# gvanhorn38/multibox

Measured on AMD Instinct MI355X. Metric: images/sec (299x299, 5-AR priors) train, higher is better.
Workload: dtype bf16; 1 GPU; full train step: Inception-ResNet-v2 + multibox heads fwd, on-device matching+loss, bwd, RMSProp+EMA; 299x299, k=5 (P=646), BATCH_SIZE=64/GPU, MAX_NUM_BBOXES=13; global_batch=64, parallelism=dp1, hip_graph=True

## Files before the change

### include/mbx.h

```cpp
#ifndef MBX_H
#define MBX_H

#include <stddef.h>
#include <stdint.h>

#ifdef __cplusplus
extern "C" {
#endif

typedef void* mbx_stream_t;

typedef enum {
  MBX_OK = 0,
  MBX_ERR_INVALID_ARG = -1,
  MBX_ERR_UNSUPPORTED = -2,
  MBX_ERR_LAUNCH = -3,
  MBX_ERR_WORKSPACE = -4
} mbx_status;

int mbx_version(void);
const char* mbx_status_string(int status);

int mbx_priors_count(int k, const int* grids, int n_grids);

// ... 9 lines not shown
size_t mbx_match_workspace_bytes(int B, int P, int G);
int mbx_match(const float* decoded , const float* conf ,
              const float* gt , const int32_t* n_gt , float alpha,
              int B, int P, int G, int32_t* match , int32_t* status ,
              void* workspace, size_t workspace_bytes, mbx_stream_t stream);

int mbx_match_extend(const float* priors , const float* gt ,
                     const int32_t* n_gt , const int32_t* status ,
                     float iou_threshold, int B, int P, int G,
                     int32_t* match ,
                     int32_t* n_extra , mbx_stream_t stream);

size_t mbx_loss_workspace_bytes(int B);
int mbx_loss_fwd_bwd(const float* decoded , const float* conf_in ,
                     int conf_is_logit, const float* gt ,
                     const int32_t* match , float alpha, float grad_scale, int B, int P,
                     int G, float* loss2 ,
                     float* d_raw_locs , float* d_logits ,
                     void* workspace, size_t workspace_bytes, mbx_stream_t stream);

size_t mbx_loss_mined_workspace_bytes(int B, int P);
int mbx_loss_fwd_bwd_mined(const float* decoded , const float* conf_in ,
                           int conf_is_logit, const float* gt ,
                           const int32_t* match , float alpha, float grad_scale, int B, int P,
                           int G, float* loss2 ,
                           float* d_raw_locs , float* d_logits ,
                           int neg_per_pos, int min_neg, int32_t* n_neg ,
                           void* workspace, size_t workspace_bytes, mbx_stream_t stream);

size_t mbx_loss_focal_workspace_bytes(int B, int P);
int mbx_loss_fwd_bwd_focal(const float* decoded , const float* conf_in ,
                           int conf_is_logit, const float* gt ,
                           const int32_t* match , float alpha, float grad_scale, int B, int P,
                           int G, float* loss2 ,
                           float* d_raw_locs , float* d_logits ,
                           float gamma, float w_pos, float w_neg,
                           int neg_per_pos , int min_neg, int32_t* n_neg ,
                           void* workspace, size_t workspace_bytes, mbx_stream_t stream);

enum { MBX_LOC_L2 = 0, MBX_LOC_SMOOTH_L1 = 1, MBX_LOC_GIOU = 2, MBX_LOC_DIOU = 3, MBX_LOC_CIOU = 4 };
size_t mbx_loss_loc_workspace_bytes(int B, int P);
int mbx_loss_fwd_bwd_loc(const float* decoded , const float* conf_in ,
                         int conf_is_logit, const float* gt ,
                         const int32_t* match , float alpha, float grad_scale, int B, int P,
                         int G, float* loss2 ,
                         float* d_raw_locs , float* d_logits ,
                         int loc_type , float loc_beta ,
                         float gamma, float w_pos, float w_neg,
                         int neg_per_pos , int min_neg, int32_t* n_neg ,
                         void* workspace, size_t workspace_bytes, mbx_stream_t stream);

typedef struct {
  int32_t offset_y, offset_x;
  int32_t patch_h, patch_w;
  int32_t image_h, image_w;
  int32_t is_flipped;
  int32_t max_to_keep;
  float restrictions[4];
} mbx_patch_meta;

int mbx_decode_filter_topk(const float* raw_locs , const float* conf ,
                           const float* priors , const mbx_patch_meta* meta ,
                           int B, int P, int k_max, double* out_boxes ,
                           float* out_scores , int32_t* out_index ,
                           int32_t* out_count , mbx_stream_t stream);

int mbx_nms(double* boxes , float* scores , int32_t* index ,
            int32_t* count , int B, int k_max, double iou_threshold, mbx_stream_t stream);

#define MBX_MERGE_MAX_CANDIDATES 16384
int mbx_merge_detections(const double* boxes , const float* scores ,
                         const int32_t* count , const int32_t* image_rows , int I, int k_max,
                         int max_det, double iou_threshold, double* out_boxes ,
                         float* out_scores , int32_t* out_src ,
                         int32_t* out_count , int32_t* out_status , mbx_stream_t stream);

int mbx_merge_detections_voted(const double* boxes , const float* scores ,
                               const int32_t* count , const int32_t* image_rows , int I,
                               int k_max, int max_det, double iou_threshold, double vote_iou_threshold,
                               double* out_boxes , float* out_scores ,
                               int32_t* out_src , int32_t* out_count ,
                               int32_t* out_status , int32_t* out_votes , mbx_stream_t stream);

#define MBX_SOFT_LINEAR 1
#define MBX_SOFT_GAUSSIAN 2
int mbx_merge_detections_soft(const double* boxes , const float* scores ,
                              const int32_t* count , const int32_t* image_rows , int I, int k_max,
                              int max_det, int method, double iou_threshold , double sigma ,
                              double min_score, double vote_iou_threshold ,
                              double* out_boxes , float* out_scores ,
                              int32_t* out_src , int32_t* out_count , int32_t* out_status ,
                              int32_t* out_votes , mbx_stream_t stream);

#define MBX_COCO_MAX_DET 100
#define MBX_COCO_MAX_GT 128
int mbx_coco_match(const double* dt , const int32_t* dt_rows ,
                   const double* gt , const int32_t* gt_rows , int I,
                   const double* iou_thrs , int T, const double* area_rng ,
                   int A, int16_t* match , uint8_t* ignore ,
                   int32_t* n_gt_counted , int32_t* status , mbx_stream_t stream);

#define MBX_COCO_ACC_MAX_R 128
#define MBX_COCO_ACC_MAX_M 4
#define MBX_COCO_ACC_MAX_ND 4194304
#define MBX_COCO_ACC_CHUNK 256
#define MBX_COCO_ACC_SORT_TILE 1024
size_t mbx_coco_accumulate_workspace(long long ND, int T, int A, int M);
int mbx_coco_accumulate(const double* dt , const int32_t* dt_rows , int I,
                        const int16_t* match , const uint8_t* ignore ,
                        const int32_t* n_gt_counted , int T, int A, const double* rec_thrs , int R,
                        const int32_t* max_dets , int M, double* precision ,
                        double* recall , void* workspace, size_t workspace_bytes, mbx_stream_t stream);

typedef enum {
  MBX_EPI_STORE = 0,
  MBX_EPI_AFFINE = 1,
  MBX_EPI_RESIDUAL = 2,
  MBX_EPI_STORE_F32 = 3
} mbx_epilogue;

typedef struct {
  int32_t n, rows_mod;
  int32_t c_begin[4];
  const void* y[4]; int32_t ld_y[4];
  const float* relu_thr[4];
  float* stats[4]; int32_t stats_ld[4];
} mbx_bn_bwd_stats;

#define MBX_GRID_BARRIER_BYTES 6400
typedef struct {
  void* barrier;
  void* a; int32_t ld_a;
  const float* beta;
  float* mean; float* rstd;
  float* moving_mean; float* moving_var;
  float* relu_thr;
  int32_t relu; float eps, decay;
  float* step_poison;
} mbx_bn_apply_desc;

#define MBX_BN_BWD_SLOTS 8
typedef struct {
  void* barrier;
  int32_t n;
  int32_t c_begin[4];
  const void* y[4]; int32_t ld_y[4];
  void* dy[4]; int32_t ld_dy[4];
  const float* mean[4]; const float* rstd[4]; const float* beta[4];
  float* dbeta[4];
  float* acc[4]; int32_t acc_ld[4];
  int32_t relu[4];
  float* step_poison;
} mbx_bn_bwd_fused;

typedef struct {
  const void* x; int64_t x_img_stride; int32_t ldx;
  int32_t N, H_in, W_in, C_in;
  const void* w; int32_t C_out, R, S;
  int32_t stride, transposed, pad_t, pad_l, H_out, W_out;
  void* y; int64_t y_img_stride; int32_t ldy;
  int32_t epilogue, relu, accumulate;
  const float* scale; const float* shift;
  const void* skip; int64_t skip_img_stride; int32_t ld_skip; float rscale;
  float* stats_partial;
  int32_t tile_config;
  const void* acc_src; int64_t acc_img_stride; int32_t ld_acc;
  int32_t* work_counter;
  int32_t max_workgroups;
  void* splitk_ws; int64_t splitk_ws_bytes;
  int32_t stats_rows_mod, stats_ld;
  const mbx_bn_bwd_stats* bn_bwd_stats;
  void* relu_bits; int32_t ld_bits;
  const mbx_bn_apply_desc* bn_apply;
  const mbx_bn_bwd_fused* bn_bwd;
} mbx_conv_desc;
#define MBX_CONV_TILE_CONFIGS 14
#define MBX_TILE_I5_BASE 32
#define MBX_TILE_I7 65
#define MBX_TILE_DIRECT3 96
#define MBX_TILE_DIRECTW 97
#define MBX_TILE_RESIDENT 98
#define MBX_TILE_PWRES 99
#define MBX_TILE_SPLITK_BASE 128
#define MBX_TILE_SPLITK_MAX 32

int mbx_conv_stats_rows(const mbx_conv_desc* desc );
int mbx_conv(const mbx_conv_desc* desc , mbx_stream_t stream);
int mbx_conv_supported(const mbx_conv_desc* desc );
int mbx_conv_pair(const mbx_conv_desc* a , const mbx_conv_desc* b , mbx_stream_t stream);
size_t mbx_conv_splitk_workspace_bytes(const mbx_conv_desc* desc );

int mbx_conv_wgrad(const mbx_conv_desc* desc , const void* dy,
                   int64_t dy_img_stride, int32_t ld_dy, float* dw, float* db, mbx_stream_t stream);

typedef struct {
  mbx_conv_desc desc;
  const void* dy; int64_t dy_img_stride; int32_t ld_dy;
  float scale;
  float* dw; float* db;
} mbx_wgrad_job;
typedef struct {
  int32_t n_layers, n_items;
  int64_t layers_off, items_off;
  int64_t queues_off, heads_off;
  double flops;
  int64_t tally_off;
} mbx_wgrad_plan_info;
#define MBX_WGRAD_DETERMINISTIC 1
#define MBX_WGRAD_SCATTER 2
size_t mbx_wgrad_plan_bytes(const mbx_wgrad_job* jobs , int n_jobs, int flags);
int mbx_wgrad_plan(const mbx_wgrad_job* jobs , int n_jobs, int flags, void* host_image, size_t bytes,
                   mbx_wgrad_plan_info* info );
int mbx_conv_wgrad_grouped(void* device_image , const mbx_wgrad_plan_info* info ,
                           mbx_stream_t stream);
int mbx_conv_wgrad_grouped_capped(void* device_image, const mbx_wgrad_plan_info* info , int max_workgroups,
                                  mbx_stream_t stream);

int mbx_conv_wgrad_scaled(const mbx_conv_desc* desc, const void* dy, int64_t dy_img_stride,
                          int32_t ld_dy, float scale, float* dw, float* db, mbx_stream_t stream);

int mbx_bn_finalize(const float* stats_partial , int rows, int C, int64_t count,
                    float eps, float decay, float* mean , float* rstd ,
                    float* moving_mean , float* moving_var ,
                    mbx_stream_t stream);
int mbx_bn_apply(const void* y, int64_t M, int C, const float* mean, const float* rstd,
                 const float* beta, int relu, void* a, int ld_a, mbx_stream_t stream);
int mbx_bn_apply_fused(const float* stats_partial, int rows, int64_t count, float eps, float decay,
                       const void* y, int64_t M, int C, const float* beta, int relu, void* a, int ld_a,
                       float* mean, float* rstd, float* moving_mean, float* moving_var,
                       mbx_stream_t stream);
int mbx_bn_apply_fused_mapped(const void* stats_fixed, int rows, int64_t count, float eps, float decay,
                              const void* y, int64_t M, int C, const float* beta, int relu, void* a, int ld_a,
                              const struct mbx_chan_map_s* a_map , float* mean, float* rstd, float* moving_mean,
                              float* moving_var, float* relu_thr, mbx_stream_t stream);
int mbx_bn_moving_update(float* moving_mean, float* moving_var, const float* batch_mean, const float* batch_var,
                         int64_t n, float decay, const float* skip_ctl, uint64_t* skipped_steps,
                         float* ema_mean, float* ema_var, float ema_decay, mbx_stream_t stream);
typedef struct mbx_chan_map_s { int32_t n; int32_t c_begin[4]; int32_t offset[4]; } mbx_chan_map;
int mbx_bn_finalize_parts(const float* const* parts , const int32_t* rows ,
                          const int32_t* Cs , int n_parts, int64_t count, float eps, float decay, float* mean,
                          float* rstd, float* moving_mean, float* moving_var, mbx_stream_t stream);
int mbx_bn_apply_mapped(const void* y, int64_t M, int C, const float* mean, const float* rstd, const float* beta,
                        int relu, void* a, int ld_a, const mbx_chan_map* a_map , mbx_stream_t stream);
int mbx_bn_apply_maxpool(const void* y, int N, int H, int W, int C, const float* mean, const float* rstd, const float* beta,
                         int relu, void* p, int64_t p_img_stride, int ld_p, int Ho, int Wo, uint8_t* argmax,
                         mbx_stream_t stream);
int mbx_bn_fold(const float* moving_mean, const float* moving_var, const float* beta, float eps,
                int C, float* scale, float* shift, mbx_stream_t stream);
int mbx_bn_bwd_rows(int64_t M, int C);
int mbx_bn_bwd_reduce(const void* da, int ld_da, const void* a, int ld_a, int relu, const void* y,
                      int64_t M, int C, const float* mean, const float* rstd, const float* beta,
                      float* partial , mbx_stream_t stream);
int mbx_bn_bwd_finalize(const float* partial, int rows, int C, int64_t M, float* dbeta ,
                        float* m12 , mbx_stream_t stream);
int mbx_bn_bwd_apply(const void* da, int ld_da, const void* a, int ld_a, int relu, const void* y,
                     int64_t M, int C, const float* mean, const float* rstd, const float* beta,
                     const float* m12, void* dy , mbx_stream_t stream);

int mbx_bn_bwd_reduce_mapped(const void* da, int ld_da, const void* a, int ld_a, int relu, const void* y, int64_t M, int C,
                             const float* mean, const float* rstd, const float* beta, float* partial,
                             const mbx_chan_map* da_map , mbx_stream_t stream);
int mbx_bn_bwd_apply_mapped(const void* da, int ld_da, const void* a, int ld_a, int relu, const void* y, int64_t M, int C,
                            const float* mean, const float* rstd, const float* beta, const float* m12, void* dy,
                            const mbx_chan_map* da_map , mbx_stream_t stream);

int mbx_bn_bwd_apply_rows(const float* stats, int rows, const void* da, int ld_da, const void* y, int64_t M, int C,
                          const float* mean, const float* rstd, const float* relu_thr, float* dbeta, void* dy,
                          const mbx_chan_map* da_map , mbx_stream_t stream);

size_t mbx_bn_bwd_onepass_workspace_bytes(int C);
int mbx_bn_bwd_onepass_supported(int64_t M, int C, int max_workgroups);
int mbx_bn_bwd_onepass(const void* da, int ld_da, int relu, const void* y, int64_t M, int C,
                       const float* mean, const float* rstd, const float* beta, float* dbeta ,
                       void* dy , void* ws, int max_workgroups, float* step_poison ,
                       mbx_stream_t stream);

int mbx_bn_bwd_rows_pooled(int N, int H, int W, int C);
int mbx_bn_bwd_reduce_pooled(const void* gy, int64_t gy_img_stride, int ld_gy, const uint8_t* argmax, int N, int H, int W,
                             int Ho, int Wo, int relu, const void* y, int C, const float* mean, const float* rstd,
                             const float* beta, float* partial , mbx_stream_t stream);
int mbx_bn_bwd_apply_pooled(const void* gy, int64_t gy_img_stride, int ld_gy, const uint8_t* argmax, int N, int H, int W,
                            int Ho, int Wo, int relu, const void* y, int C, const float* mean, const float* rstd,
                            const float* beta, const float* m12, void* dy, mbx_stream_t stream);
int mbx_bn_bwd_onepass_mapped(const void* da, int ld_da, int relu, const void* y, int64_t M, int C, const float* mean,
                              const float* rstd, const float* beta, float* dbeta, void* dy, void* ws, int max_workgroups,
                              float* step_poison, const mbx_chan_map* da_map , mbx_stream_t stream);

int mbx_maxpool_fwd(const void* x, int64_t x_img_stride, int ldx, int N, int H, int W, int C,
                    int k, int stride, void* y, int64_t y_img_stride, int ldy, int Ho, int Wo,
                    uint8_t* argmax , mbx_stream_t stream);
int mbx_maxpool_bwd(const void* dy, int64_t dy_img_stride, int ld_dy, const uint8_t* argmax,
                    int N, int H, int W, int C, int k, int stride, int Ho, int Wo, void* dx,
                    int64_t dx_img_stride, int ld_dx, int accumulate, mbx_stream_t stream);
int mbx_avgpool_fwd(const void* x, int64_t x_img_stride, int ldx, int N, int H, int W, int C,
                    int k, int pad, void* y, int64_t y_img_stride, int ldy, int Ho, int Wo,
                    mbx_stream_t stream);
int mbx_avgpool_bwd(const void* dy, int64_t dy_img_stride, int ld_dy, int N, int H, int W, int C,
                    int k, int pad, int Ho, int Wo, void* dx, int64_t dx_img_stride, int ld_dx,
                    int accumulate, mbx_stream_t stream);

int mbx_relu_mask(void* g, int ld_g, const void* a, int ld_a, int64_t M, int C, mbx_stream_t stream);
int mbx_pack_input(const float* img, int64_t pixels, void* out, mbx_stream_t stream);
int mbx_head_gather(const float* h, int ld_h, int N, int cells, int k, int P, int off,
                    float* locs, float* logits, mbx_stream_t stream);
int mbx_head_scatter(const float* d_locs, const float* d_logits, int N, int cells, int k, int P,
                     int off, void* g, int ld_g, mbx_stream_t stream);

typedef struct {
  const float* h; int32_t ld_h;
  void* g; int32_t ld_g;
  int32_t cells, k, off;
} mbx_head;
int mbx_head_gather_all(const mbx_head* heads , int n_heads, int N, int P, float* locs, float* logits,
                        mbx_stream_t stream);
int mbx_head_scatter_all(const float* d_locs, const float* d_logits, const mbx_head* heads , int n_heads, int N,
                         int P, mbx_stream_t stream);

int mbx_step_begin(float* grads, int64_t n_grads, float* bn_ws, int64_t n_ws, int64_t ctl_index, uint64_t* timeouts_total,
                   float* zero_scalar, mbx_stream_t stream);

typedef struct {
  int64_t src_off;
  int64_t dst_off;
  int32_t K, R, S, C, Kpad;
  int32_t first_block;
} mbx_filter_entry;
int mbx_filter_prepare(const void* w_bf16, void* w_dgrad, const mbx_filter_entry* table ,
// ... 56 lines not shown
```

### multibox_amd/csrc/conv.hip

```cpp
#include <stdlib.h>

#include "conv_common.h"

namespace {

template <int BM, int BN, int WNW, int WMW, int EV, int MODE = 0, int NSTG = 3>
__device__ __forceinline__ void conv_igemm3_body(const ConvK& p, const int bid_, const int nblk_) {
  constexpr bool SH = MODE == 2, PW = MODE == 1;
  static_assert(WNW * WMW == 4 || WNW * WMW == 8, "four or eight waves");
  constexpr int NT = 64 * WNW * WMW, RPP = NT / 8;
  constexpr int TN = BN / WNW, TM = BM / WMW, NI = TN / 16, MI = TM / 16;
  constexpr int PI = BM / RPP, WI = BN / RPP, NL = PI + WI;
  constexpr int STAGE = (BM + BN) * 8;
  extern __shared__ __attribute__((aligned(16))) u32x4 smem[];

  const int tid = threadIdx.x, lane = tid & 63;
  const int wave = wave_id();
  const int wn = wave % WNW, wm = wave / WNW;
  int lid = xcd_remap(bid_, nblk_);
  int split = 0;
  if constexpr (EV == 5) { const int nt = p.tiles_m * p.tiles_n; split = lid / nt; lid -= split * nt; }
  const int tile_n = lid % p.tiles_n, tile_m = lid / p.tiles_n;
  const int m0 = tile_m * BM, n0 = tile_n * BN;

// ... 394 lines not shown
  return MBX_OK;
}

}

extern "C" int mbx_conv_stats_rows(const mbx_conv_desc* d) {
  if (!d) return MBX_ERR_INVALID_ARG;
  if (d->stats_rows_mod > 0) return d->stats_rows_mod;
  const long M = (long)d->N * d->H_out * d->W_out;
  if (d->tile_config > kSplitFlag) return (int)((M + kSplitRows - 1) / kSplitRows);
  if (d->tile_config == kDirectCfg) return mbx_direct3_grid(d->N, d->H_out, d->W_out);
  if (d->tile_config == kDirectWCfg) { const int g = mbx_directw_grid(d->N, d->H_out, d->W_out); return g > 0 ? g : MBX_ERR_UNSUPPORTED; }
  if (d->tile_config == kResidentCfg) return mbx_resident_rows(d->N);
  if (d->tile_config == kI7Cfg) return (int)((M + 127) / 128);
  if (d->tile_config > kI5Flag) {
    const int i = d->tile_config - kI5Flag - 1;
    if (i >= mbx_i5_num_tiles) return MBX_ERR_INVALID_ARG;
    return (int)((M + mbx_i5_tiles[i][0] - 1) / mbx_i5_tiles[i][0]);
  }
  const TileCfg& c = kCfgs[choose_cfg(M, d->C_out, d->tile_config)];
  return (int)((M + c.BM - 1) / c.BM);
}

static int conv_impl(const mbx_conv_desc* d, mbx_stream_t stream, int dry);
extern "C" int mbx_conv(const mbx_conv_desc* d, mbx_stream_t stream) { return conv_impl(d, stream, 0); }
extern "C" int mbx_conv_supported(const mbx_conv_desc* d) { return conv_impl(d, nullptr, 1); }
extern "C" int mbx_conv_pair(const mbx_conv_desc* a, const mbx_conv_desc* b, mbx_stream_t stream) {
  PairCapture ca, cb;
  g_capture.valid = 0;
  int st = conv_impl(a, stream, 2);
  if (st != MBX_OK) return st;
  if (!g_capture.valid) return MBX_ERR_UNSUPPORTED;
  ca = g_capture;
  g_capture.valid = 0;
  st = conv_impl(b, stream, 2);
  if (st != MBX_OK) return st;
  if (!g_capture.valid) return MBX_ERR_UNSUPPORTED;
  cb = g_capture;
  if (ca.bm != cb.bm || ca.bn != cb.bn || ca.wnw != cb.wnw || ca.wmw != cb.wmw || ca.nstg != cb.nstg || ca.ev != cb.ev ||
      ca.mode != 0 || cb.mode != 0 || (ca.ev != 0 && ca.ev != 1 && ca.ev != 6) || ca.wnw != 2 || ca.wmw != 2 || ca.bn != 64)
    return MBX_ERR_UNSUPPORTED;
  ca.k.dry = cb.k.dry = 0;
  hipStream_t s = mbx_s(stream);
#define MBX_PAIR(BM_, NSTG_)                                                                                      \
  if (ca.bm == BM_ && ca.nstg == NSTG_)                                                                           \
    return ca.ev == 6 ? launch_pair_inst<BM_, 64, 2, 2, 6, NSTG_>(ca.k, cb.k, s)                                    \
           : ca.ev ? launch_pair_inst<BM_, 64, 2, 2, 1, NSTG_>(ca.k, cb.k, s) : launch_pair_inst<BM_, 64, 2, 2, 0, NSTG_>(ca.k, cb.k, s);
  MBX_PAIR(128, 2) MBX_PAIR(128, 3) MBX_PAIR(64, 2) MBX_PAIR(64, 3)
#undef MBX_PAIR
  return MBX_ERR_UNSUPPORTED;
}

extern "C" size_t mbx_conv_splitk_workspace_bytes(const mbx_conv_desc* d) {
  if (!d || d->tile_config <= kSplitFlag || d->tile_config > kSplitFlag + kSplitMax) return 0;
  int ksplit, kps;
  splitk_geom((d->R * d->S * d->C_in + 63) >> 6, d->tile_config - kSplitFlag, ksplit, kps);
  return (size_t)4 * d->N * d->H_out * d->W_out * (((d->C_out + 7) / 8) * 8) * ksplit;
}

static int conv_impl(const mbx_conv_desc* d, mbx_stream_t stream, int dry) {
  int st = check_desc(d);
  if (st != MBX_OK) return st;
  if (!d->w || !d->y) return MBX_ERR_INVALID_ARG;
  if ((reinterpret_cast<uintptr_t>(d->w) & 15)) return MBX_ERR_INVALID_ARG;
  const bool f32 = d->epilogue == MBX_EPI_STORE_F32;
  if (!f32 && (d->C_out % 8 || d->ldy % 8 || (reinterpret_cast<uintptr_t>(d->y) & 15))) return MBX_ERR_INVALID_ARG;
  if (d->epilogue == MBX_EPI_RESIDUAL && (!d->skip || d->ld_skip % 8 || (reinterpret_cast<uintptr_t>(d->skip) & 15)))
    return MBX_ERR_INVALID_ARG;
  if ((long long)d->N * d->y_img_stride >= (1LL << 31)) return MBX_ERR_UNSUPPORTED;
  if (d->stats_partial && (d->epilogue != MBX_EPI_STORE || d->accumulate || d->skip)) return MBX_ERR_INVALID_ARG;
  if (d->epilogue == MBX_EPI_STORE && d->skip && (d->ld_skip % 8 || (reinterpret_cast<uintptr_t>(d->skip) & 15))) return MBX_ERR_INVALID_ARG;
  MBX_ENTER();
  ConvK k;
  k.x = reinterpret_cast<const unsigned short*>(d->x);
  k.x_img_stride = (int)d->x_img_stride; k.ldx = d->ldx; k.H_in = d->H_in; k.W_in = d->W_in; k.C_in = d->C_in;
  k.w = reinterpret_cast<const unsigned short*>(d->w);
  k.C_out = d->C_out; k.R = d->R; k.S = d->S; k.Ktot = d->R * d->S * d->C_in;
  k.x_bytes = (unsigned)(2 * ((long long)(d->N - 1) * d->x_img_stride + ((long long)d->H_in * d->W_in - 1) * d->ldx + d->C_in));
  k.w_bytes = (unsigned)(2LL * d->C_out * k.Ktot);
  if (d->transposed) { k.mul = 1; k.shift = d->stride == 2 ? 1 : 0; } else { k.mul = d->stride; k.shift = 0; }
  k.pad_t = d->pad_t; k.pad_l = d->pad_l; k.W_out = d->W_out; k.HW_out = d->H_out * d->W_out;
  k.M = d->N * k.HW_out;
  k.y = d->y; k.y_img_stride = (int)d->y_img_stride; k.ldy = d->ldy;
  k.epi = d->epilogue; k.relu = d->relu; k.accumulate = d->accumulate;
  k.scale = d->scale; k.shiftv = d->shift;
  k.skip = reinterpret_cast<const unsigned short*>(d->skip);
  k.skip_img_stride = (int)d->skip_img_stride; k.ld_skip = d->ld_skip; k.rscale = d->rscale;
  k.bits = nullptr; k.bits_ld = 0; k.bits_bytes = 0;
  if (d->relu_bits) {
    const bool wr = d->epilogue == MBX_EPI_RESIDUAL && d->relu, rd = d->epilogue == MBX_EPI_STORE && !d->skip;
    if ((!wr && !rd) || d->ld_bits % 4 || d->ld_bits < 4 * ((d->C_out + 31) / 32) || (reinterpret_cast<uintptr_t>(d->relu_bits) & 3)) return MBX_ERR_INVALID_ARG;
    if (d->stats_partial || d->bn_bwd_stats) return MBX_ERR_UNSUPPORTED;
    const long long bb = (long long)d->N * d->H_out * d->W_out * d->ld_bits;
    if (bb >= (1LL << 31)) return MBX_ERR_UNSUPPORTED;
    k.bits = reinterpret_cast<unsigned char*>(d->relu_bits); k.bits_ld = d->ld_bits; k.bits_bytes = (unsigned)bb;
  }
  k.stats = d->stats_partial;
  if (d->stats_rows_mod < 0 || d->stats_rows_mod > 1024 || d->stats_ld < 0 || (d->stats_ld && d->stats_ld < d->C_out)) return MBX_ERR_INVALID_ARG;
  k.stats_mod = d->stats_rows_mod; k.stats_ld = d->stats_ld ? d->stats_ld : d->C_out;
  k.stats_cap = 0.f;
  k.fa = FusedApply{};
  k.fa.bar = nullptr;
  k.fb = FusedBwd{};
  k.fb.bar = nullptr;
  if (d->bn_bwd) {
    const mbx_bn_bwd_fused* b = d->bn_bwd;
    if (!b->barrier || (reinterpret_cast<uintptr_t>(b->barrier) & 127) || b->n < 1 || b->n > 4 || b->c_begin[0] != 0) return MBX_ERR_INVALID_ARG;
    if (d->epilogue != MBX_EPI_STORE || d->accumulate || d->skip || d->relu_bits || d->stats_partial || d->bn_bwd_stats || d->bn_apply ||
        d->stride != 1 || d->C_out > 2048 || d->y_img_stride != (int64_t)d->H_out * d->W_out * d->ldy)
      return MBX_ERR_UNSUPPORTED;
    const int tc = d->tile_config;
    if (!((tc > kI5Flag && tc <= kI5Flag + 7) || tc == kDirectWCfg || tc == kResidentCfg)) return MBX_ERR_UNSUPPORTED;
    const long long Mll = (long long)d->N * d->H_out * d->W_out;
    for (int i = 0; i < 4; ++i) k.fb.cb[i] = 1 << 30;
    for (int i = 0; i < b->n; ++i) {
      if (!b->y[i] || !b->dy[i] || !b->mean[i] || !b->rstd[i] || (b->relu[i] && !b->beta[i]) || !b->acc[i] ||
          (reinterpret_cast<uintptr_t>(b->y[i]) & 15) || (reinterpret_cast<uintptr_t>(b->dy[i]) & 15) || b->ld_y[i] % 8 || b->ld_dy[i] % 8 ||
          b->c_begin[i] % 8 || b->c_begin[i] >= d->C_out || (i && b->c_begin[i] <= b->c_begin[i - 1]) || b->acc_ld[i] <= 0)
        return MBX_ERR_INVALID_ARG;
      if (Mll * b->ld_y[i] >= (1LL << 31) || Mll * b->ld_dy[i] >= (1LL << 31)) return MBX_ERR_UNSUPPORTED;
      k.fb.cb[i] = b->c_begin[i];
      k.fb.y[i] = reinterpret_cast<const unsigned short*>(b->y[i]); k.fb.ldy[i] = b->ld_y[i];
      k.fb.dy[i] = reinterpret_cast<unsigned short*>(b->dy[i]); k.fb.lddy[i] = b->ld_dy[i];
      k.fb.mean[i] = b->mean[i]; k.fb.rstd[i] = b->rstd[i]; k.fb.beta[i] = b->beta[i]; k.fb.dbeta[i] = b->dbeta[i];
      k.fb.acc[i] = b->acc[i]; k.fb.acc_ld[i] = b->acc_ld[i]; k.fb.relu[i] = b->relu[i];
    }
    const int fault = mbx_barrier_fault() == '3';
    k.fb.n = b->n;
    k.fb.bar = reinterpret_cast<unsigned*>(b->barrier);
    static const int probe = mbx_env_int("MBX_FUSED_PROBE", 0) & ~1;
    k.fb.spin_limit = fault ? (1u << 10) : (1u << 22); k.fb.fault = fault | probe; k.fb.step_poison = b->step_poison;
    k.fb.inv_M = (float)(1.0 / (double)Mll);
  }
  if (d->bn_apply) {
    const mbx_bn_apply_desc* b = d->bn_apply;
    if (!b->barrier || !b->a || !b->beta || !b->mean || !b->rstd || (reinterpret_cast<uintptr_t>(b->barrier) & 127) ||
        (reinterpret_cast<uintptr_t>(b->a) & 15) || b->ld_a % 8 || b->ld_a < d->C_out)
      return MBX_ERR_INVALID_ARG;
    if (!d->stats_partial || d->stats_rows_mod < 1 || d->stats_rows_mod > 16 || d->epilogue != MBX_EPI_STORE || d->accumulate || d->skip ||
        d->transposed || d->rscale != 0.f || d->C_out > 2048 || d->y_img_stride != (int64_t)d->H_out * d->W_out * d->ldy ||
        (long long)d->N * d->H_out * d->W_out * b->ld_a >= (1LL << 31))
      return MBX_ERR_UNSUPPORTED;
    const int tc = d->tile_config;
    if (!((tc > kI5Flag && tc <= kI5Flag + 7) || tc == kDirectWCfg || tc == kResidentCfg)) return MBX_ERR_UNSUPPORTED;
    const int fault = mbx_barrier_fault() == '2';
    k.fa.bar = reinterpret_cast<unsigned*>(b->barrier);
    static const int probe = mbx_env_int("MBX_FUSED_PROBE", 0) & ~1;
    k.fa.spin_limit = fault ? (1u << 10) : (1u << 22); k.fa.fault = fault | probe; k.fa.step_poison = b->step_poison;
    k.fa.a = reinterpret_cast<unsigned short*>(b->a); k.fa.ld_a = b->ld_a; k.fa.beta = b->beta;
    k.fa.mean = b->mean; k.fa.rstd = b->rstd; k.fa.mmean = b->moving_mean; k.fa.mvar = b->moving_var; k.fa.thr = b->relu_thr;
    k.fa.relu = b->relu; k.fa.eps = b->eps; k.fa.decay = b->decay;
    k.fa.inv_count = 1.0 / (double)((long long)d->N * d->H_out * d->W_out);
  }
  k.bw_n = 0; k.bw_mod = 1;
  for (int i = 0; i < 4; ++i) { k.bw_cb[i] = 1 << 30; k.bw_ldy[i] = 0; k.bw_sld[i] = 0; k.bw_y[i] = nullptr; k.bw_thr[i] = nullptr; k.bw_stats[i] = nullptr; }
  if (d->bn_bwd_stats) {
    const mbx_bn_bwd_stats* b = d->bn_bwd_stats;
    if (d->epilogue != MBX_EPI_STORE || d->accumulate || d->skip || d->stats_partial || b->n < 1 || b->n > 4 || b->rows_mod < 1 ||
        b->rows_mod > 1024 || b->c_begin[0] != 0)
      return MBX_ERR_INVALID_ARG;
    for (int i = 0; i < b->n; ++i) {
      if (!b->y[i] || !b->relu_thr[i] || !b->stats[i] || (reinterpret_cast<uintptr_t>(b->y[i]) & 15) || b->ld_y[i] % 8 || b->c_begin[i] % 32 ||
          b->c_begin[i] >= d->C_out || (i && b->c_begin[i] <= b->c_begin[i - 1]) || b->stats_ld[i] <= 0)
        return MBX_ERR_INVALID_ARG;
      k.bw_cb[i] = b->c_begin[i]; k.bw_ldy[i] = b->ld_y[i]; k.bw_sld[i] = b->stats_ld[i];
      k.bw_y[i] = reinterpret_cast<const unsigned short*>(b->y[i]); k.bw_thr[i] = b->relu_thr[i]; k.bw_stats[i] = b->stats[i];
    }
    k.bw_n = b->n; k.bw_mod = b->rows_mod;
  }
  if (d->accumulate && d->acc_src) {
    if (d->ld_acc % 8 || (reinterpret_cast<uintptr_t>(d->acc_src) & 15) || (long long)d->N * d->acc_img_stride >= (1LL << 31))
      return MBX_ERR_INVALID_ARG;
    k.acc_src = reinterpret_cast<const unsigned short*>(d->acc_src); k.acc_img_stride = (int)d->acc_img_stride; k.ld_acc = d->ld_acc;
  } else {
    k.acc_src = reinterpret_cast<const unsigned short*>(d->y); k.acc_img_stride = (int)d->y_img_stride; k.ld_acc = d->ldy;
  }
  {
    const long long last_pix = (long long)k.HW_out - 1, span = ((d->C_out + 7) / 8) * 8;
    const long long yb = 2 * ((long long)(d->N - 1) * d->y_img_stride + last_pix * d->ldy + span);
    const long long sb = d->skip ? 2 * ((long long)(d->N - 1) * d->skip_img_stride + last_pix * d->ld_skip + span) : 0;
    const long long ab = 2 * ((long long)(d->N - 1) * k.acc_img_stride + last_pix * k.ld_acc + span);
    if (!f32 && (yb >= (1LL << 31) || sb >= (1LL << 31) || ab >= (1LL << 31))) return MBX_ERR_UNSUPPORTED;
    k.y_bytes = (unsigned)yb; k.skip_bytes = (unsigned)sb; k.acc_bytes = (unsigned)ab;
  }
  set_magic((unsigned)k.HW_out, k.mg_hw, k.sh_hw);
  set_magic((unsigned)k.W_out, k.mg_w, k.sh_w);
  k.pw = (d->R == 1 && d->S == 1 && d->pad_t == 0 && d->pad_l == 0 && d->stride == 1) ? 1 : 0;
  k.skip_taps = 0; k.parity = 0;
  k.work_counter = d->work_counter;
  k.max_wg = d->max_workgroups;
  k.dry = dry;
  k.ksplit = 1; k.kps = 1 << 30; k.y_split_stride = 0;
#ifdef MBX_I5_STAMPS
  {
    static const unsigned long long sp = getenv("MBX_I5_STAMP_PTR") ? strtoull(getenv("MBX_I5_STAMP_PTR"), nullptr, 10) : 0ull;
    k.stamps = reinterpret_cast<unsigned long long*>(sp);
    k.dbg = mbx_env_int("MBX_I5_DBG", 0);
    k.stagger = mbx_env_int("MBX_STAGGER", 0);
  }
#endif
  for (int c = 0; c < 4; ++c) { k.cls_m0[c] = 0; k.cls_hw[c] = 1; k.cls_w[c] = 1; }
  static const bool notap = mbx_env_char("MBX_NO_TAP_SKIP") == '1';
  if (k.shift && d->C_in % 64 == 0 && !notap) {
    int m0 = 0;
    for (int c = 0; c < 4; ++c) {
      const int hc = (d->H_out - (c >> 1) + 1) / 2, wc = (d->W_out - (c & 1) + 1) / 2;
      k.cls_m0[c] = m0;
      k.cls_hw[c] = hc * wc > 0 ? hc * wc : 1;
      k.cls_w[c] = wc > 0 ? wc : 1;
      m0 += d->N * hc * wc;
    }
    k.skip_taps = k.parity = 1;
  }
  if (k.bits && k.shift) return MBX_ERR_UNSUPPORTED;
  hipStream_t s = mbx_s(stream);
  if (d->tile_config > kSplitFlag) {
    const int S = d->tile_config - kSplitFlag;
    if (S < 2 || S > kSplitMax || d->transposed || d->bn_bwd_stats || d->relu_bits || d->epilogue != MBX_EPI_STORE || d->accumulate || d->skip || d->rscale != 0.f)
      return MBX_ERR_UNSUPPORTED;
    const int ldp = ((d->C_out + 7) / 8) * 8;
    int ksplit, kps;
    splitk_geom((k.Ktot + 63) >> 6, S, ksplit, kps);
    const long long slice = (long long)k.M * ldp;
    if (!d->splitk_ws || (reinterpret_cast<uintptr_t>(d->splitk_ws) & 15) || d->splitk_ws_bytes < (int64_t)(4 * slice * ksplit) ||
        slice * ksplit >= (1LL << 31))
      return MBX_ERR_WORKSPACE;
    ConvK g = k;
    g.epi = MBX_EPI_STORE_F32; g.stats = nullptr; g.relu = 0;
    g.y = d->splitk_ws; g.ldy = ldp; g.y_img_stride = k.HW_out * ldp;
    g.ksplit = ksplit; g.kps = kps; g.y_split_stride = slice;
    st = launch_igemm<128, 64, 2, 2>(g, s);
    if (st != MBX_OK || dry) return st;
    hipLaunchKernelGGL(splitk_reduce_kernel, dim3((k.M + kSplitRows - 1) / kSplitRows), dim3(256), 0, s, reinterpret_cast<const float*>(d->splitk_ws),
                       ksplit, slice, k.M, k.C_out, ldp, reinterpret_cast<unsigned short*>(k.y), k.HW_out,
                       (long long)k.y_img_stride, k.ldy, k.stats, k.stats_mod, k.stats_ld, stats_cap_for((k.M + kSplitRows - 1) / kSplitRows));
    MBX_LAUNCH_CHECK();
    return MBX_OK;
  }
  if (d->tile_config == kDirectCfg) return mbx_launch_direct3(k, d->N, d->H_out, s);
  if (d->tile_config == kDirectWCfg) return mbx_launch_directw(k, d->N, d->H_out, s);
  if (d->tile_config == kResidentCfg) return mbx_launch_resident(k, d->N, d->H_out, s);
  if (d->tile_config == kPwResCfg) return mbx_launch_pwres(k, s);
  if (d->tile_config == kI7Cfg) return mbx_launch_igemm7(k, s);
  if (d->tile_config > kI5Flag) return mbx_launch_igemm5(k, d->tile_config - kI5Flag - 1, s);
  switch (choose_cfg(k.M, k.C_out, d->tile_config)) {
    case 0: return launch_igemm<128, 128, 2, 2>(k, s);
    case 1: return launch_igemm<128, 64, 2, 2>(k, s);
    case 2: return launch_igemm<64, 128, 2, 2>(k, s);
    case 3: return launch_igemm<128, 32, 1, 4>(k, s);
    case 5: return launch_igemm<256, 128, 2, 4>(k, s);
    case 6: return launch_igemm<128, 128, 2, 4>(k, s);
    case 7: return launch_igemm<256, 64, 1, 8>(k, s);
    case 8: return launch_igemm<128, 128, 2, 4, 2>(k, s);
    case 9: return launch_igemm<128, 64, 2, 2, 2>(k, s);
    case 10: return launch_igemm<64, 64, 2, 2, 2>(k, s);
    case 11: return launch_igemm<128, 64, 2, 4, 2>(k, s);
    case 12: return launch_igemm<256, 64, 1, 8, 2>(k, s);
    case 13: return launch_igemm<128, 128, 2, 2, 2>(k, s);
    default: return launch_igemm<64, 64, 2, 2>(k, s);
  }
}
```

### multibox_amd/csrc/conv_common.h

```cpp
#pragma once
#include <type_traits>
#include "common.h"
#include "grid_barrier.h"

namespace mbx {

struct ConvK {
  const unsigned short* x; int x_img_stride, ldx, H_in, W_in, C_in;
  const unsigned short* w; int C_out, R, S, Ktot;
  unsigned x_bytes, w_bytes;
  unsigned y_bytes, skip_bytes, acc_bytes;
  int mul, shift, pad_t, pad_l, W_out, HW_out, M;
  void* y; int y_img_stride, ldy;
  int epi, relu, accumulate;
  const float* scale; const float* shiftv;
  const unsigned short* skip; int skip_img_stride, ld_skip; float rscale;
  const unsigned short* acc_src; int acc_img_stride, ld_acc;
  unsigned char* bits; int bits_ld; unsigned bits_bytes;
  float* stats;
  float stats_cap;
  int stats_mod, stats_ld;
  int bw_n, bw_mod;
  int bw_cb[4], bw_ldy[4], bw_sld[4];
  const unsigned short* bw_y[4];
  const float* bw_thr[4];
  float* bw_stats[4];
  FusedApply fa;
  FusedBwd fb;
  int tiles_m, tiles_n;
  unsigned mg_hw, sh_hw, mg_w, sh_w;
  int pw;
  int cls_m0[4], cls_hw[4], cls_w[4];
  int skip_taps;
  int parity;
  int* work_counter;
  int max_wg;
  int dry;
  int ksplit, kps; long long y_split_stride;
#ifdef MBX_I5_STAMPS
  unsigned long long* stamps;
  int dbg;
  int stagger;
#endif
};

}

int mbx_launch_igemm5(mbx::ConvK& k, int index, hipStream_t s);
extern const int mbx_i5_tiles[][2];
extern const int mbx_i5_num_tiles;
int mbx_launch_igemm7(mbx::ConvK& k, hipStream_t s);
int mbx_launch_direct3(mbx::ConvK& k, int N, int H_out, hipStream_t s);
int mbx_direct3_grid(int N, int H_out, int W_out);
int mbx_launch_directw(mbx::ConvK& k, int N, int H_out, hipStream_t s);
int mbx_directw_grid(int N, int H_out, int W_out);
int mbx_launch_resident(mbx::ConvK& k, int N, int H_out, hipStream_t s);
int mbx_resident_rows(int N);
int mbx_launch_pwres(mbx::ConvK& k, hipStream_t s);

namespace {

using mbx::ConvK;
using mbx::FusedApply;
using mbx::FusedBwd;

typedef __attribute__((ext_vector_type(8))) __bf16 bf16x8;
typedef __attribute__((ext_vector_type(4))) float f32x4;
typedef __attribute__((ext_vector_type(4))) short s16x4;
typedef __attribute__((ext_vector_type(4))) unsigned int u32x4;
typedef __attribute__((ext_vector_type(2))) unsigned int u32x2;

__device__ __forceinline__ float bf2f(unsigned short h) { return __uint_as_float(((unsigned)h) << 16); }
__device__ __forceinline__ unsigned short f2bf(float f) { return __builtin_bit_cast(unsigned short, (__bf16)f); }
typedef float f32x4u __attribute__((ext_vector_type(4), aligned(4)));
__device__ __forceinline__ unsigned pack2bf(float lo, float hi) {
  typedef float pk_f32x2 __attribute__((ext_vector_type(2)));
  typedef __bf16 pk_bf16x2 __attribute__((ext_vector_type(2)));
  return __builtin_bit_cast(unsigned, __builtin_convertvector(pk_f32x2{lo, hi}, pk_bf16x2));
}
__device__ __forceinline__ float bf_lo(unsigned w) { return __uint_as_float(w << 16); }
__device__ __forceinline__ float bf_hi(unsigned w) { return __uint_as_float(w & 0xffff0000u); }
__device__ __forceinline__ unsigned gather4_rows(unsigned b) {
  typedef unsigned g4_u32x2 __attribute__((ext_vector_type(2)));
  const g4_u32x2 r = __builtin_amdgcn_permlane16_swap(b, b, false, false);
  const unsigned t = r.x | (r.y << 8);
  const g4_u32x2 q = __builtin_amdgcn_permlane32_swap(t, t, false, false);
  return q.x | (q.y << 16);
}
__device__ __forceinline__ float relu_f(float x) {
  float r;
  asm("v_max_f32 %0, 0, %1" : "=v"(r) : "v"(x));
  return r;
}

constexpr int kThreads = 256;

inline int conv_cus() { const int n = mbx_cu_count(); return n ? n : 256; }

inline bool store_or_affine_only(const ConvK& k) {
  return (k.epi == MBX_EPI_STORE || k.epi == MBX_EPI_AFFINE) && !k.accumulate && !k.skip && !k.bits && k.rscale == 0.f && !k.bw_n &&
         !(k.epi == MBX_EPI_AFFINE && k.stats);
}

template <typename Q, typename F>
inline int launch_by_ev(const ConvK& k, const Q& q, int grid, int threads, int lds, hipStream_t s, F kern) {
  static bool attr[3] = {false, false, false};
  const int ev = k.epi == MBX_EPI_AFFINE ? 2 : k.stats ? 1 : 0;
  void (*const fn)(const ConvK, const Q) = ev == 2 ? kern(std::integral_constant<int, 3>())
                                           : ev   ? kern(std::integral_constant<int, 1>()) : kern(std::integral_constant<int, 0>());
  if (!attr[ev]) {
    (void)hipFuncSetAttribute(reinterpret_cast<const void*>(fn), hipFuncAttributeMaxDynamicSharedMemorySize, lds);
    attr[ev] = true;
  }
  hipLaunchKernelGGL(fn, dim3(grid), dim3(threads), lds, s, k, q);
  MBX_LAUNCH_CHECK();
  return MBX_OK;
}

inline void set_magic(unsigned d, unsigned& mg, unsigned& sh) {
  unsigned l = 0;
  while ((1ull << l) < d) ++l;
  sh = 31 + l;
  mg = (unsigned)((1ull << sh) / d + 1);
}

inline int check_desc(const mbx_conv_desc* d) {
  if (!d || !d->x || !d->N || d->N < 0) return MBX_ERR_INVALID_ARG;
  if (d->C_in <= 0 || d->C_in % 8 || d->ldx % 8 || d->ldx < d->C_in) return MBX_ERR_INVALID_ARG;
  if (d->R <= 0 || d->S <= 0 || d->C_out <= 0 || d->H_out <= 0 || d->W_out <= 0) return MBX_ERR_INVALID_ARG;
  if (d->stride != 1 && d->stride != 2) return MBX_ERR_UNSUPPORTED;
  if ((reinterpret_cast<uintptr_t>(d->x) & 15)) return MBX_ERR_INVALID_ARG;
  const long long xe = (long long)d->N * d->x_img_stride;
  if (xe >= (1LL << 30) || (long long)d->N * d->H_out * d->W_out >= (1LL << 31)) return MBX_ERR_UNSUPPORTED;
  return MBX_OK;
}

__device__ __forceinline__ float row_sum16(float v) {
  asm volatile("s_nop 1\n\t"
               "v_add_f32_dpp %0, %0, %0 row_ror:8 row_mask:0xf bank_mask:0xf\n\t"
               "s_nop 1\n\t"
               "v_add_f32_dpp %0, %0, %0 row_ror:4 row_mask:0xf bank_mask:0xf\n\t"
               "s_nop 1\n\t"
               "v_add_f32_dpp %0, %0, %0 row_ror:2 row_mask:0xf bank_mask:0xf\n\t"
               "s_nop 1\n\t"
               "v_add_f32_dpp %0, %0, %0 row_ror:1 row_mask:0xf bank_mask:0xf"
               : "+v"(v));
  return v;
}
__device__ __forceinline__ void row_sum16_x8(float (&v)[8]) {
#define MBX_RS_STEP(R)                                                                                                     \
  "v_add_f32_dpp %0, %0, %0 row_ror:" #R " row_mask:0xf bank_mask:0xf\n\tv_add_f32_dpp %1, %1, %1 row_ror:" #R " row_mask:0xf bank_mask:0xf\n\t" \
  "v_add_f32_dpp %2, %2, %2 row_ror:" #R " row_mask:0xf bank_mask:0xf\n\tv_add_f32_dpp %3, %3, %3 row_ror:" #R " row_mask:0xf bank_mask:0xf\n\t" \
  "v_add_f32_dpp %4, %4, %4 row_ror:" #R " row_mask:0xf bank_mask:0xf\n\tv_add_f32_dpp %5, %5, %5 row_ror:" #R " row_mask:0xf bank_mask:0xf\n\t" \
  "v_add_f32_dpp %6, %6, %6 row_ror:" #R " row_mask:0xf bank_mask:0xf\n\tv_add_f32_dpp %7, %7, %7 row_ror:" #R " row_mask:0xf bank_mask:0xf\n\t"
  asm volatile("s_nop 1\n\t" MBX_RS_STEP(8) MBX_RS_STEP(4) MBX_RS_STEP(2) MBX_RS_STEP(1)
               : "+v"(v[0]), "+v"(v[1]), "+v"(v[2]), "+v"(v[3]), "+v"(v[4]), "+v"(v[5]), "+v"(v[6]), "+v"(v[7]));
#undef MBX_RS_STEP
}
__device__ __forceinline__ unsigned fast_div(unsigned m, unsigned magic, unsigned shift) {
  return (unsigned)(((unsigned long long)m * magic) >> shift);
}
constexpr float kStatsFix = 1048576.f;
constexpr float kStatsTotal = 4398046511104.f;
__host__ __device__ __forceinline__ float stats_cap_for(long long adders) { return kStatsTotal / (float)(adders > 0 ? adders : 1); }
__device__ __forceinline__ void stats_add_fixed(unsigned long long* o, const float x1, const float x2, const float cap) {
  if (__builtin_fabsf(x1) < cap && __builtin_fabsf(x2) < cap) {
    atomicAdd(o, (unsigned long long)__float2ll_rn(x1 * kStatsFix));
    atomicAdd(o + 1, (unsigned long long)__float2ll_rn(x2 * kStatsFix));
  } else {
    atomicMin(reinterpret_cast<long long*>(o + 1), (long long)0x8000000000000000ull);
  }
}
__device__ __forceinline__ void stats_write(const ConvK& p, const int tile_row, const int ch, const float x1, const float x2) {
  if (p.stats_mod) {
    unsigned long long* o = reinterpret_cast<unsigned long long*>(p.stats) + ((size_t)(tile_row % p.stats_mod) * p.stats_ld + ch) * 2;
    stats_add_fixed(o, x1, x2, p.stats_cap);
  } else {
    float* o = p.stats + ((size_t)tile_row * p.stats_ld + ch) * 2;
    o[0] = x1;
    o[1] = x2;
  }
}
__device__ __forceinline__ int bw_seg(const ConvK& p, const int c) {
  int s = 0;
#pragma unroll
  for (int i = 1; i < 4; ++i) if (i < p.bw_n && c >= p.bw_cb[i]) s = i;
  return s;
}
__device__ __forceinline__ void bw_stats_write(const ConvK& p, const int tile_row, const int ch, const float x1, const float x2) {
  const int s = bw_seg(p, ch);
  float* o = p.bw_stats[s] + ((size_t)(tile_row % p.bw_mod) * p.bw_sld[s] + (ch - p.bw_cb[s])) * 2;
  unsafeAtomicAdd(o, x1);
  unsafeAtomicAdd(o + 1, x2);
}
__device__ __forceinline__ void decode_pixel(const ConvK& p, unsigned m, int& img, int& oh, int& ow) {
  img = (int)fast_div(m, p.mg_hw, p.sh_hw);
  const int rem = (int)m - img * p.HW_out;
  oh = (int)fast_div((unsigned)rem, p.mg_w, p.sh_w);
  ow = rem - oh * p.W_out;
}
__device__ __forceinline__ void decode_pixel_parity(const ConvK& p, unsigned m, int& img, int& oh, int& ow) {
  const int c = ((int)m >= p.cls_m0[1]) + ((int)m >= p.cls_m0[2]) + ((int)m >= p.cls_m0[3]);
  const int m0 = c == 0 ? p.cls_m0[0] : c == 1 ? p.cls_m0[1] : c == 2 ? p.cls_m0[2] : p.cls_m0[3];
  const int hw = c == 0 ? p.cls_hw[0] : c == 1 ? p.cls_hw[1] : c == 2 ? p.cls_hw[2] : p.cls_hw[3];
  const int wc = c == 0 ? p.cls_w[0] : c == 1 ? p.cls_w[1] : c == 2 ? p.cls_w[2] : p.cls_w[3];
  unsigned r = m - (unsigned)m0;
  img = (int)(r / (unsigned)hw);
  r -= (unsigned)img * (unsigned)hw;
  const int a = (int)(r / (unsigned)wc), b = (int)r - a * wc;
  oh = 2 * a + (c >> 1);
  ow = 2 * b + (c & 1);
}
__device__ __forceinline__ int pixel_class(const ConvK& p, int m) {
  return (m >= p.cls_m0[1]) + (m >= p.cls_m0[2]) + (m >= p.cls_m0[3]);
}
constexpr unsigned kOOB = 0x80000000u;

// ... 288 lines not shown
```

### multibox_amd/csrc/convr.hip

```cpp
#include "direct_epilogue.h"
#ifndef MBX_RES_EALL
#define MBX_RES_EALL 0
#endif
#ifndef MBX_RES_PROBE
#define MBX_RES_PROBE 0
#endif

namespace {

constexpr int kRThreads = 512;
constexpr int kRCW = 4, kRLW = 4;

struct ResK {
  int N, H, W, HW;
  int NG, CPT;
  int ntiles;
  int per;
  int npi;
  int dh[9], dw[9], dd[9];
};

template <int C8>
__device__ __forceinline__ int rkey(int r) {
  return (C8 % 16 == 0) ? 2 * (r & 7) : (C8 % 16 == 8) ? 2 * ((r >> 1) & 3) : 2 * ((r >> 2) & 1);
}
template <int C8> constexpr int rjx() { return (C8 % 16 == 0) ? 3 : (C8 % 16 == 8) ? 1 : 0; }
template <int C8>
__device__ __forceinline__ int renc(int row, int fch) {
  const int k = rkey<C8>(row);
  return row * C8 + (fch ^ (k & 3)) + 4 * (k >> 2);
}
template <int C8>
__device__ __forceinline__ int rslot(int E, int j) { return (E ^ (4 * (j & rjx<C8>()))) + 4 * (j & ~rjx<C8>()); }
template <int C8>
__device__ __forceinline__ int rencb(int row, int fch, int base) { return base + 16 * renc<C8>(row, fch); }
typedef const __attribute__((address_space(3))) u32x4* lds_u32x4_cptr;
__device__ __forceinline__ int lds_addr(const void* p) { return (int)(unsigned)(size_t)((const __attribute__((address_space(3))) char*)p); }
template <int C8>
__device__ __forceinline__ bf16x8 rread(int Eb, int j) {
  const unsigned a = (unsigned)((Eb ^ (64 * (j & rjx<C8>()))) + 64 * (j & ~rjx<C8>()));
  return __builtin_bit_cast(bf16x8, *(lds_u32x4_cptr)(size_t)a);
}

template <int PT>
__device__ __forceinline__ void wait_vmcnt_k(const int k) {
  switch (k) {
    case 0: wait_vmcnt<0>(); break;
    case 1: wait_vmcnt<PT>(); break;
    case 2: wait_vmcnt<2 * PT>(); break;
    case 3: wait_vmcnt<3 * PT>(); break;
    case 4: wait_vmcnt<4 * PT>(); break;
    case 5: wait_vmcnt<5 * PT>(); break;
    case 6: wait_vmcnt<6 * PT>(); break;
    case 7: wait_vmcnt<(7 * PT < 63 ? 7 * PT : 0)>(); break;
    default: wait_vmcnt<0>(); break;
  }
}


template <int NR, int NM, int I = 0>
__device__ __forceinline__ void sched_interleave() {
  if constexpr (I < NR) {
    __builtin_amdgcn_sched_group_barrier(0x100, 1, 0);
    __builtin_amdgcn_sched_group_barrier(0x008, I + 1 < NR ? 1 : NM - (NR - 1), 0);
    sched_interleave<NR, NM, I + 1>();
  }
}

template <int C8, int NB, int RS, int MI>
struct ResG {
  static constexpr int HWMAX = 16 * kRCW * MI;
  static constexpr int KC = C8 / 4;
  static constexpr int SLOT_CH = NB * 16 * C8;
  static constexpr int PT = (SLOT_CH + 64 * kRLW - 1) / (64 * kRLW);
  static constexpr int SLOTP = PT * kRLW * 64;
  static constexpr int RED_CH = kRCW * NB * 16 * 2 * 4 / 16;
  static constexpr int img_ch(int hw) { return ((hw + 1) * C8 + 63) / 64 * 64; }
  static constexpr int lds_bytes(int hw, int d) { return (RED_CH + d * SLOTP + img_ch(hw)) * 16; }
  static constexpr int depth(int hw) {
    int d = RS;
    while (d > 2 && lds_bytes(hw, d) > 160 * 1024) --d;
    return d;
  }
};

template <int C8, int NB, int RS, int MI, int HWC, int EV>
__global__ void __launch_bounds__(kRThreads)
conv_resident_kernel(const ConvK p, const ResK q) {
  using G = ResG<C8, NB, RS, MI>;
  constexpr int KC = G::KC, PT = G::PT, SLOTP = G::SLOTP, D = G::depth(HWC), DD = D < RS ? D : RS;
  constexpr int GR = D >= RS ? (RS < 4 ? RS : 4) : (D / 2 > 0 ? D / 2 : 1), G0 = GR < RS ? GR : RS;
  static_assert(D >= RS || D >= 2 * GR || GR == 1, "two groups in the ring");
  extern __shared__ __attribute__((aligned(16))) u32x4 smem[];
  float* const red = reinterpret_cast<float*>(smem);
  u32x4* const ring = smem + G::RED_CH;
  u32x4* const img = ring + D * SLOTP;

  const int tid = threadIdx.x, lane = tid & 63;
  const int wave = wave_id();
  const __amdgpu_buffer_rsrc_t xr = make_rsrc(p.x, p.x_bytes);
  const __amdgpu_buffer_rsrc_t wr = make_rsrc(p.w, p.w_bytes);
  const int first = xcd_remap((int)blockIdx.x, (int)gridDim.x);
  const int frow = lane & 15, fch = lane >> 4;

  auto issue_image = [&](const int im) {
    const int xo = im * p.x_img_stride;
    for (int i = wave; i < q.npi; i += 8) {
      const int ci = i * 64 + lane;
      const int pix = ci / C8, cs = ci - pix * C8;
      const int c = cs ^ rkey<C8>(pix);
      glds16(xr, img + i * 64, pix < q.HW ? (xo + pix * p.ldx + c * 8) * 2 : (int)kOOB);
    }
  };

  if (wave >= kRCW) {
    const int lw = wave - kRCW;
    int wo[PT];
    bool wv[PT];
    int rowch[PT];
#pragma unroll
    for (int i = 0; i < PT; ++i) {
      const int ci = (lw + kRLW * i) * 64 + lane;
      const int row = ci / C8, cs = ci - row * C8;
      const int c = cs ^ rkey<C8>(row);
      wv[i] = row < 16 * NB;
      rowch[i] = wv[i] ? dperm<16 * NB>(row >> 4, row & 15) : 0;
      wo[i] = (rowch[i] * RS * (8 * C8) + c * 8) * 2;
    }
    int im_in = -1, base = 0;
    const int t0 = first * q.per, t1 = min(t0 + q.per, q.ntiles);
    for (int t = t0; t < t1; ++t) {
      const int im = t / q.NG;
      const bool last = t + 1 == t1;
      auto issue_tap = [&](const int rel) {
        const int tt = rel < RS ? t : t + 1, tap = rel < RS ? rel : rel - RS;
        const int g = tt - (tt / q.NG) * q.NG;
        const int cb = g * q.CPT, ce = min(cb + q.CPT, p.C_out);
        const int wbase = cb * RS * (8 * C8) * 2;
        const int sl = D == RS ? tap : (base + rel) % D;
        u32x4* dst = ring + sl * SLOTP + lw * 64;
#pragma unroll
        for (int i = 0; i < PT; ++i)
          glds16(wr, dst + i * (kRLW * 64), (wv[i] && cb + rowch[i] < ce) ? wbase + wo[i] + tap * (8 * C8) * 2 : (int)kOOB);
      };
      auto slot_of = [&](const int rel) { return D == RS ? rel % RS : (base + rel) % D; };
      if (t == t0) {
        issue_image(im);
#pragma unroll
        for (int tap = 0; tap < DD; ++tap) issue_tap(tap);
        wait_vmcnt_k<PT>(DD - G0);
      } else if (im != im_in) {
        issue_image(im);
        wait_vmcnt<0>();
      } else {
        wait_vmcnt_k<PT>(DD - G0);
      }
      im_in = im;
      lds_readback_wait(lds_readback_issue(ring + slot_of(G0 - 1) * SLOTP + (PT - 1) * (kRLW * 64) + lw * 64 + lane));
      raw_barrier();
#pragma unroll
      for (int g0 = 0; g0 < RS; g0 += GR) {
        const int e = g0 + GR < RS ? g0 + GR : RS;
        if (e < RS) {
          const int e2 = e + GR < RS ? e + GR : RS;
          if (last) wait_vmcnt_k<PT>((DD + g0 < RS ? DD + g0 : RS) - e2);
          else wait_vmcnt_k<PT>(DD + g0 - e2);
          lds_readback_wait(lds_readback_issue(ring + slot_of(e2 - 1) * SLOTP + (PT - 1) * (kRLW * 64) + lw * 64 + lane));
        }
        raw_barrier();
#pragma unroll
        for (int k2 = g0; k2 < e; ++k2)
          if (DD + k2 < RS || !last) issue_tap(DD + k2);
      }
      if constexpr (EV == 1) raw_barrier();
      if constexpr (D != RS) base = (base + RS) % D;
    }
  } else {
  const __amdgpu_buffer_rsrc_t yr = make_rsrc(p.y, p.y_bytes);
  constexpr int RING_OFF0 = G::RED_CH * 16, IMG_OFF0 = RING_OFF0 + D * SLOTP * 16;
  const int RING_OFF = RING_OFF0 + lds_addr(smem), IMG_OFF = IMG_OFF0 + lds_addr(smem);
  static_assert(RING_OFF0 % 256 == 0 && (SLOTP * 16) % 256 == 0, "the XOR-ed address bits of a row must be clear in the region offsets");
  int EA[NB];
#pragma unroll
  for (int a = 0; a < NB; ++a) EA[a] = rencb<C8>(16 * a + frow, fch, RING_OFF);
  constexpr bool EALL = MBX_RES_EALL;
  int E[EALL ? RS : 2][MI];
  int opix[MI], vm[MI];
#pragma unroll
  for (int f = 0; f < MI; ++f) {
    const int pl = 16 * (wave + kRCW * f) + frow;
    const bool pv = pl < q.HW;
    opix[f] = pv ? pl : -1;
    const int oh = pv ? (int)fast_div((unsigned)pl, p.mg_w, p.sh_w) : -(1 << 20);
    const int ow = pv ? pl - oh * q.W : 0;
    int m = 0;
#pragma unroll
    for (int tap = 0; tap < RS; ++tap)
      m |= ((int)((unsigned)(oh + q.dh[tap]) < (unsigned)q.H) & (int)((unsigned)(ow + q.dw[tap]) < (unsigned)q.W)) << tap;
    vm[f] = m;
  }
  auto tap_rows = [&](const int tap, int (&e)[MI]) {
#pragma unroll
    for (int f = 0; f < MI; ++f) e[f] = rencb<C8>((vm[f] & (1 << tap)) ? opix[f] + q.dd[tap] : q.HW, fch, IMG_OFF);
  };
#ifdef MBX_I5_STAMPS
  const bool stamp = p.stamps && tid == 0 && blockIdx.x < 64;
#define MBXR_STAMP(i) do { if (stamp && t == first * q.per + p.dbg) p.stamps[(blockIdx.x * 8) * 4 + (i)] = wall_clock64(); } while (0)
#else
#define MBXR_STAMP(i) do { } while (0)
#endif
  int im_in = -1, base = 0;
  for (int t = first * q.per, t1 = min(t + q.per, q.ntiles); t < t1; ++t) {
    const int im = t / q.NG, g = t - im * q.NG;
    const int cb = g * q.CPT, ce = min(cb + q.CPT, p.C_out);
    const bool newim = im != im_in;
    im_in = im;
    MBXR_STAMP(0);
    if (newim) issue_image(im);
    DirAffine<NB> af;
    direct_affine_load<EV, NB>(p, cb, ce, fch, af);
    if constexpr (EALL) {
#pragma unroll
      for (int tap = 0; tap < RS; ++tap) tap_rows(tap, E[tap]);
    } else {
      tap_rows(0, E[0]);
    }
    if (newim) {
      wait_vmcnt<0>();
      lds_readback_wait(lds_readback_issue(img + lane));
    }
    raw_barrier();
    MBXR_STAMP(1);
#pragma unroll
    for (int a = 0; a < NB; ++a) asm volatile("" : "+v"(EA[a]));
#pragma unroll
    for (int f = 0; f < MI; ++f) asm volatile("" : "+v"(opix[f]), "+v"(vm[f]));

    f32x4 acc[NB][MI];
#pragma unroll
    for (int a = 0; a < NB; ++a)
#pragma unroll
      for (int f = 0; f < MI; ++f) acc[a][f] = f32x4{0.f, 0.f, 0.f, 0.f};
    constexpr int NS = RS * KC, NR = NB + MI, NM = NB * MI;
    int sofs[RS];
#pragma unroll
    for (int tap = 0; tap < RS; ++tap) sofs[tap] = (D == RS ? tap : (base + tap) % D) * (SLOTP * 16);
    if constexpr (D != RS) base = (base + RS) % D;
    bf16x8 wf[2][NB], pf[2][MI];
#pragma unroll
    for (int a = 0; a < NB; ++a) wf[0][a] = rread<C8>(EA[a] + sofs[0], 0);
#pragma unroll
    for (int f = 0; f < MI; ++f) pf[0][f] = rread<C8>(E[0][f], 0);
    __builtin_amdgcn_sched_barrier(0);
#pragma unroll
    for (int s = 0; s < NS; ++s) {
      const int cur = s & 1, nxt = cur ^ 1;
      const int tap1 = (s + 1) / KC, j1 = (s + 1) % KC;
      if (j1 == 0 && (tap1 % GR == 0 || tap1 == RS)) {
        asm volatile("s_waitcnt lgkmcnt(0)" ::: "memory");
        raw_barrier();
        __builtin_amdgcn_sched_barrier(0);
      }
      if constexpr (!EALL) { if (s % KC == 0 && s / KC + 1 < RS) tap_rows(s / KC + 1, E[(s / KC + 1) & 1]); }
      constexpr bool rd_ = !(MBX_RES_PROBE & 1), mm_ = !(MBX_RES_PROBE & 2);
      if (s + 1 < NS && rd_) {
        const int so = sofs[tap1 < RS ? tap1 : 0];
#pragma unroll
        for (int a = 0; a < NB; ++a) wf[nxt][a] = rread<C8>(EA[a] + so, j1);
#pragma unroll
        for (int f = 0; f < MI; ++f) pf[nxt][f] = rread<C8>(E[EALL ? (tap1 < RS ? tap1 : 0) : (tap1 & 1)][f], j1);
      }
      if (mm_) {
#pragma unroll
      for (int f = 0; f < MI; ++f)
#pragma unroll
        for (int a = 0; a < NB; ++a)
          acc[a][f] = __builtin_amdgcn_mfma_f32_16x16x32_bf16(wf[cur][a], pf[cur][f], acc[a][f], 0, 0, 0);
      }
      if (s + 1 < NS) sched_interleave<NR, NM>();
      __builtin_amdgcn_sched_barrier(0);
    }

    MBXR_STAMP(2);
    float s1[NB][4], s2[NB][4];
#pragma unroll
    for (int a = 0; a < NB; ++a)
#pragma unroll
      for (int r = 0; r < 4; ++r) { s1[a][r] = 0.f; s2[a][r] = 0.f; }
    const int yo = im * p.y_img_stride;
#pragma unroll
    for (int f = 0; f < MI; ++f) {
      const bool pv = opix[f] >= 0;
      direct_store_pixel<EV>(p, yr, acc, f, pv, yo + (pv ? opix[f] : 0) * p.ldy, cb, ce, fch, af, s1, s2);
    }
    if constexpr (EV == 1) {
      {
        float v[NB * 8];
#pragma unroll
        for (int a = 0; a < NB; ++a)
#pragma unroll
          for (int r = 0; r < 4; ++r) { v[a * 8 + r] = s1[a][r]; v[a * 8 + 4 + r] = s2[a][r]; }
#pragma unroll
        for (int a = 0; a < NB; ++a) {
          float u[8] = {v[a * 8], v[a * 8 + 1], v[a * 8 + 2], v[a * 8 + 3], v[a * 8 + 4], v[a * 8 + 5], v[a * 8 + 6], v[a * 8 + 7]};
          row_sum16_x8(u);
          if (frow == 0) {
#pragma unroll
            for (int r = 0; r < 4; ++r) {
              const int ch = dperm<16 * NB>(a, 4 * fch + r);
              red[(wave * 16 * NB + ch) * 2] = u[r];
              red[(wave * 16 * NB + ch) * 2 + 1] = u[4 + r];
            }
          }
        }
      }
      lds_barrier();
      if (tid < 16 * NB && cb + tid < ce) {
        float x1 = 0.f, x2 = 0.f;
#pragma unroll
        for (int w = 0; w < kRCW; ++w) { x1 += red[(w * 16 * NB + tid) * 2]; x2 += red[(w * 16 * NB + tid) * 2 + 1]; }
        stats_write(p, im, cb + tid, x1, x2);
      }
    }
    MBXR_STAMP(3);
  }
#undef MBXR_STAMP
  }
  if constexpr (EV == 1) {
    if (p.fa.bar != nullptr) {
      fused_apply_tail<kRThreads>(p, ring, [&](auto&& fn) {
        for (int t = first * q.per, t1 = min(t + q.per, q.ntiles); t < t1; ++t) {
          const int im = t / q.NG, g = t - im * q.NG;
          const int cb = g * q.CPT, ce = min(cb + q.CPT, p.C_out);
          fn(im * q.HW, q.HW, cb, ce - cb);
        }
      });
    }
  }
  if constexpr (EV == 0) {
    if (p.fb.bar != nullptr) {
      static_assert(kRThreads * 68 + sizeof(FbShared) <= (G::depth(HWC) * SLOTP + G::img_ch(HWC)) * 16, "the tail's reduce area fits ring + image");
      fused_bwd_tail<kRThreads, false>(p, ring, [&](auto&& fn) {
        for (int t = first * q.per, t1 = min(t + q.per, q.ntiles); t < t1; ++t) {
          const int im = t / q.NG, g = t - im * q.NG;
          const int cb = g * q.CPT, ce = min(cb + q.CPT, p.C_out);
          fn(im * q.HW, q.HW, cb, ce - cb);
        }
      });
    }
  }
}

struct PwK {
  int npt, NCS, nct, ctper, nunits;
  int npi;
};
constexpr int kPwCol = 128;

template <int C8, int MIH>
struct PwG {
  static constexpr int PIX = 32 * MIH;
  static constexpr int KC = C8 / 4;
  static constexpr int PIX_CH = (PIX * C8 + 63) / 64 * 64;
  static constexpr int ROOM = 160 * 1024 / 16 - PIX_CH;
  static constexpr int KS = (C8 % 8 == 0 && ROOM / (kPwCol * 8) >= 3) ? 2 : 1;
  static constexpr int NSL = KC / KS;
  static constexpr int C8S = 4 * KS;
  static constexpr int SLOT_CH = kPwCol * C8S;
  static constexpr int PT = SLOT_CH / (64 * kRLW);
  static constexpr int NST_RAW = ROOM / SLOT_CH;
  static constexpr int NST = NST_RAW > 8 ? 8 : NST_RAW;
  static constexpr int LDS_BYTES = (NST * SLOT_CH + PIX_CH) * 16;
  static_assert(KC % KS == 0 && NST >= 3 && (NST - 1) * PT < 64, "ring");
};

template <int C8, int MIH, int EV>
__global__ void __launch_bounds__(kRThreads)
conv_pwres_kernel(const ConvK p, const PwK q) {
  using G = PwG<C8, MIH>;
  constexpr int KC = G::KC, KS = G::KS, NSL = G::NSL, C8S = G::C8S, SLOT_CH = G::SLOT_CH, PT = G::PT, NST = G::NST, PIX = G::PIX;
  constexpr int MI = 2 * MIH, NI = 2, NA = 1;
  constexpr int EVC = EV, BMODE = EV == 2 ? 2 : 1;
  extern __shared__ __attribute__((aligned(16))) u32x4 smem[];
  u32x4* const ring = smem;
// ... 52 lines not shown
      int pos1 = 1 % NST;
      for (int s_ = 0; s_ < NS; ++s_) {
        if (s_ + 1 < NS) {
          const int newer = (s_ + NST - 1 < NS - 1 ? s_ + NST - 1 : NS - 1) - (s_ + 1);
          if (newer >= NST - 2) wait_vmcnt<(NST - 2) * PT>();
          else if (NST > 3 && newer == NST - 3) wait_vmcnt<(NST - 3 > 0 ? NST - 3 : 0) * PT>();
          else if (NST > 4 && newer == NST - 4) wait_vmcnt<(NST - 4 > 0 ? NST - 4 : 0) * PT>();
          else if (NST > 5 && newer == NST - 5) wait_vmcnt<(NST - 5 > 0 ? NST - 5 : 0) * PT>();
          else if (NST > 6 && newer == NST - 6) wait_vmcnt<(NST - 6 > 0 ? NST - 6 : 0) * PT>();
          else if (NST > 7 && newer == NST - 7) wait_vmcnt<(NST - 7 > 0 ? NST - 7 : 0) * PT>();
          else wait_vmcnt<0>();
          lds_readback_wait(lds_readback_issue(ring + pos1 * SLOT_CH + (PT - 1) * (kRLW * 64) + lw * 64 + lane));
        }
        raw_barrier();
        if (si < NS) issue_slot();
        pos1 = pos1 == NST - 1 ? 0 : pos1 + 1;
      }
    }
    return;
  }

  const int lds0 = lds_addr(smem);
  int EA[NI], Ep0;
#pragma unroll
  for (int a = 0; a < NI; ++a) EA[a] = rencb<C8S>(32 * wave + 16 * a + frow, fch, lds0);
  Ep0 = rencb<C8>(frow, fch, lds0 + NST * SLOT_CH * 16);
#ifdef MBX_I5_STAMPS
  const bool stamp = p.stamps && tid == 0 && blockIdx.x < 64;
#define MBXP_STAMP(ci, i) do { if (stamp && u == first && (ci) < 8) p.stamps[(blockIdx.x * 8 + (ci)) * 4 + (i)] = wall_clock64(); } while (0)
#else
#define MBXP_STAMP(ci, i) do { } while (0)
#endif
  for (int u = first; u < q.nunits; u += G_) {
    const int pt = u / q.NCS, cs_ = u - pt * q.NCS;
    const int ct0 = cs_ * q.ctper, ct1 = min(ct0 + q.ctper, q.nct);
    const int m0 = pt * PIX;
    issue_pixels(m0);
    wait_vmcnt<0>();
    lds_readback_wait(lds_readback_issue(pix + lane));
    raw_barrier();
#pragma unroll
    for (int a = 0; a < NI; ++a) asm volatile("" : "+v"(EA[a]));
    asm volatile("" : "+v"(Ep0));
    int so = 0;
    const int mlane = m0 + frow;
    for (int ct = ct0; ct < ct1; ++ct) {
      const int clane = ct * kPwCol + 32 * wave + 8 * fch;
      MBXP_STAMP(ct - ct0, 0);
#ifdef MBX_I5_STAMPS
      const unsigned long long clk0 = __builtin_amdgcn_s_memtime();
#endif
      u32x4 la[MI][NA], lb[MI][NA];
#ifdef MBX_I5_STAMPS
      const bool epi_ = !(p.dbg & 16);
#else
      constexpr bool epi_ = true;
#endif
      if (epi_) conv_epilogue_issue_reads<EVC, false, NA, MI, BMODE>(p, mlane, clane, 0, la, lb);
      float s1[NA][8], s2[NA][8], sc[NA][8], sh[NA][8];
      conv_epilogue_channels<EVC, NA>(p, clane, sc, sh, s1, s2);
      f32x4 acc[NI][MI];
#pragma unroll
      for (int a = 0; a < NI; ++a)
#pragma unroll
        for (int f = 0; f < MI; ++f) acc[a][f] = f32x4{0.f, 0.f, 0.f, 0.f};
      bf16x8 wf[2][NI], pf[2][MIH];
#pragma unroll
      for (int a = 0; a < NI; ++a) wf[0][a] = rread<C8S>(EA[a] + so, 0);
#pragma unroll
      for (int f = 0; f < MIH; ++f) pf[0][f] = rread<C8>(Ep0 + f * (16 * C8 * 16), 0);
      __builtin_amdgcn_sched_barrier(0);
#pragma unroll
      for (int h = 0; h < 2 * KC; ++h) {
        const int s = h >> 1, half = h & 1;
        const int h1 = h + 1, s1_ = h1 >> 1, half1 = h1 & 1;
        if (half1 == 0 && s1_ % KS == 0) {
          asm volatile("s_waitcnt lgkmcnt(0)" ::: "memory");
          raw_barrier();
          so = so == (NST - 1) * SLOT_CH * 16 ? 0 : so + SLOT_CH * 16;
          __builtin_amdgcn_sched_barrier(0);
        }
#ifdef MBX_I5_STAMPS
        const bool rd_ = !(p.dbg & 4), mm_ = !(p.dbg & 8);
#else
        constexpr bool rd_ = true, mm_ = true;
#endif
        if (h1 < 2 * KC && rd_) {
          if (half1 == 0) {
#pragma unroll
            for (int a = 0; a < NI; ++a) wf[s1_ & 1][a] = rread<C8S>(EA[a] + so, s1_ % KS);
          }
#pragma unroll
          for (int f = 0; f < MIH; ++f) pf[h1 & 1][f] = rread<C8>(Ep0 + (MIH * half1 + f) * (16 * C8 * 16), s1_);
        }
        if (mm_) {
#pragma unroll
        for (int f = 0; f < MIH; ++f)
#pragma unroll
          for (int a = 0; a < NI; ++a)
            acc[a][MIH * half + f] = __builtin_amdgcn_mfma_f32_16x16x32_bf16(wf[s & 1][a], pf[h & 1][f], acc[a][MIH * half + f], 0, 0, 0);
        }
        if (h1 < 2 * KC) { if (half1 == 0) sched_interleave<NI + MIH, NI * MIH>(); else sched_interleave<MIH, NI * MIH>(); }
        __builtin_amdgcn_sched_barrier(0);
      }
      MBXP_STAMP(ct - ct0, 1);
#ifdef MBX_I5_STAMPS
      if (stamp && u == first && ct - ct0 < 8) p.stamps[(blockIdx.x * 8 + (ct - ct0)) * 4 + 3] = __builtin_amdgcn_s_memtime() - clk0;
#endif
      if (epi_) conv_epilogue_finish<EVC, false, NI, MI, MI, BMODE>(p, acc, mlane, clane, 0, la, lb, sh, sc, s1, s2);
      MBXP_STAMP(ct - ct0, 2);
    }
  }
#undef MBXP_STAMP
}

template <int C8, int MIH, int EV>
int launch_pwres(const ConvK& k, PwK& q, hipStream_t s) {
  using G = PwG<C8, MIH>;
  constexpr int lds = G::LDS_BYTES;
  static_assert(lds <= 160 * 1024, "LDS");
  q.npt = (k.M + G::PIX - 1) / G::PIX;
  q.nct = (k.C_out + kPwCol - 1) / kPwCol;
  const int ncu = conv_cus();
  int ncs = ncu / q.npt;
  if (ncs < 1) ncs = 1;
  if (ncs > q.nct) ncs = q.nct;
  q.ctper = (q.nct + ncs - 1) / ncs;
  q.NCS = (q.nct + q.ctper - 1) / q.ctper;
  q.nunits = q.npt * q.NCS;
  q.npi = G::PIX_CH / 64;
  int grid = q.nunits < ncu ? q.nunits : ncu;
  if (k.max_wg > 0 && grid > k.max_wg) grid = k.max_wg;
  if (k.dry) return MBX_OK;
  static bool attr = false;
  if (!attr) {
    (void)hipFuncSetAttribute(reinterpret_cast<const void*>(conv_pwres_kernel<C8, MIH, EV>), hipFuncAttributeMaxDynamicSharedMemorySize, lds);
    attr = true;
  }
  hipLaunchKernelGGL((conv_pwres_kernel<C8, MIH, EV>), dim3(grid), dim3(kRThreads), lds, s, k, q);
  MBX_LAUNCH_CHECK();
  return MBX_OK;
}

template <int C8, int NB, int RS, int MI, int HWC>
int launch_resident(const ConvK& k, const ResK& q, int grid, hipStream_t s) {
  using G = ResG<C8, NB, RS, MI>;
  constexpr int lds = G::lds_bytes(HWC, G::depth(HWC));
  static_assert(lds <= 160 * 1024, "LDS");
  static_assert((G::depth(HWC) - 1) * G::PT < 64, "vmcnt");
  static_assert(HWC <= G::HWMAX, "pixel slots");
  return launch_by_ev(k, q, grid, kRThreads, lds, s, [](auto ev) { return conv_resident_kernel<C8, NB, RS, MI, HWC, decltype(ev)::value>; });
}

inline void resident_groups(int C_out, int& NG, int& CPT, int& NB) {
  NG = 4;
  CPT = ((C_out + NG * 8 - 1) / (NG * 8)) * 8;
  NB = (CPT + 15) / 16;
}

}

int mbx_resident_rows(int N) { return N; }

int mbx_launch_resident(ConvK& k, int N, int H_out, hipStream_t s) {
  if (k.mul != 1 || k.shift || !store_or_affine_only(k)) return MBX_ERR_UNSUPPORTED;
  if (k.H_in != H_out || k.W_in != k.W_out || k.C_out % 8 || k.pad_t < 0 || k.pad_l < 0 || k.pad_t >= k.R || k.pad_l >= k.S)
    return MBX_ERR_UNSUPPORTED;
  ResK q;
  q.N = N; q.H = H_out; q.W = k.W_out; q.HW = H_out * k.W_out;
  int NB;
  resident_groups(k.C_out, q.NG, q.CPT, NB);
  q.ntiles = N * q.NG;
  k.stats_cap = stats_cap_for(N);
  const int C8 = k.C_in / 8, RS = k.R * k.S;
  if (k.C_in % 32 || q.HW > 289 || q.HW < 64) return MBX_ERR_UNSUPPORTED;
  q.npi = ((q.HW + 1) * C8 + 63) / 64;
  if (RS > 9) return MBX_ERR_UNSUPPORTED;
  for (int t = 0; t < 9; ++t) { q.dh[t] = q.dw[t] = q.dd[t] = 0; }
  for (int t = 0; t < RS; ++t) { q.dh[t] = t / k.S - k.pad_t; q.dw[t] = t % k.S - k.pad_l; q.dd[t] = q.dh[t] * q.W + q.dw[t]; }
  int grid = q.ntiles < conv_cus() ? q.ntiles : conv_cus();
  if (k.max_wg > 0 && grid > k.max_wg) grid = k.max_wg;
  q.per = (q.ntiles + grid - 1) / grid;
  grid = (q.ntiles + q.per - 1) / q.per;
#define MBX_RES(C8_, NB_, RS_, MI_, HWC_)                                                                \
  if (C8 == C8_ && NB == NB_ && RS == RS_ && q.HW <= HWC_ && (HWC_ > 64 || q.HW == 64)) {                 \
    if (k.dry) return MBX_OK;                                                                            \
    return launch_resident<C8_, NB_, RS_, MI_, HWC_>(k, q, grid, s);                                     \
  }
  MBX_RES(24, 4, 3, 1, 64) MBX_RES(28, 4, 3, 1, 64) MBX_RES(28, 3, 3, 1, 64) MBX_RES(32, 4, 3, 1, 64)
  if (q.HW <= 64) return MBX_ERR_UNSUPPORTED;
  MBX_RES(16, 3, 7, 5, 289) MBX_RES(20, 3, 7, 5, 289) MBX_RES(20, 2, 7, 5, 289) MBX_RES(24, 3, 7, 5, 289)
#undef MBX_RES
  return MBX_ERR_UNSUPPORTED;
}

int mbx_launch_pwres(ConvK& k, hipStream_t s) {
  if (!k.pw || k.shift || k.stats || k.bw_n || k.C_out % 8) return MBX_ERR_UNSUPPORTED;
  const bool res = k.epi == MBX_EPI_RESIDUAL, accm = k.epi == MBX_EPI_STORE && k.bits && !k.skip;
  if (!res && !accm) return MBX_ERR_UNSUPPORTED;
  PwK q;
  if (res) {
    switch (k.C_in) {
      case 96: return launch_pwres<12, 5, 4>(k, q, s);
      case 128: return launch_pwres<16, 5, 4>(k, q, s);
      case 320: return launch_pwres<40, 5, 4>(k, q, s);
      case 384: return launch_pwres<48, 5, 4>(k, q, s);
      case 448: return launch_pwres<56, 4, 4>(k, q, s);
      default: return MBX_ERR_UNSUPPORTED;
    }
  }
  switch (k.C_in) {
    case 96: return launch_pwres<12, 5, 2>(k, q, s);
    case 128: return launch_pwres<16, 4, 2>(k, q, s);
    case 320: return launch_pwres<40, 5, 2>(k, q, s);
    case 384: return launch_pwres<48, 4, 2>(k, q, s);
    case 448: return launch_pwres<56, 4, 2>(k, q, s);
    default: return MBX_ERR_UNSUPPORTED;
  }
}
```

### multibox_amd/csrc/fused_bn.h

```cpp
#pragma once
#include "grid_barrier.h"

namespace {

using mbx::FusedApply;
using mbx::FusedBwd;

constexpr int kAuxSc1 = 16;
__device__ __forceinline__ u32x4 ld16_agent(__amdgpu_buffer_rsrc_t r, unsigned byte_off) {
  return __builtin_amdgcn_raw_buffer_load_b128(r, (int)byte_off, 0, kAuxSc1);
}
__device__ __forceinline__ float ld4_agent(__amdgpu_buffer_rsrc_t r, unsigned byte_off) {
  return __builtin_bit_cast(float, __builtin_amdgcn_raw_buffer_load_b32(r, (int)byte_off, 0, kAuxSc1));
}
constexpr int kProbeNoWait = 16, kProbeNoTotals = 32, kProbeNoSweep = 64, kProbeNoSums = 128;

template <int NT>
__device__ __forceinline__ void fused_stats_to_lds(const FusedApply& f, const float* stats, const int rows, const int ld, const int C,
                                                   float* s_par, const bool timed_out) {
  const __amdgpu_buffer_rsrc_t sr = make_rsrc(stats, (f.fault & kProbeNoTotals) ? 0u : (unsigned)(rows * ld * 16));
  for (int ch = threadIdx.x; ch < C; ch += NT) {
    u32x4 v[16];
#pragma unroll
    for (int r = 0; r < 16; ++r) v[r] = ld16_agent(sr, r < rows ? (unsigned)((r * ld + ch) * 16) : kOOB);
    const float be = f.beta[ch];
    long long i1 = 0, i2 = 0;
    bool bad = false;
#pragma unroll
    for (int r = 0; r < 16; ++r) {
      const long long v1 = (long long)(((unsigned long long)v[r].y << 32) | v[r].x), v2 = (long long)(((unsigned long long)v[r].w << 32) | v[r].z);
      i1 += v1; i2 += v2;
      bad |= v2 < 0;
    }
    const double s1 = (double)i1 * (1.0 / 1048576.0), s2 = (double)i2 * (1.0 / 1048576.0);
    const double mu = s1 * f.inv_count;
    double var = s2 * f.inv_count - mu * mu;
    if (var < 0.0) var = 0.0;
    const bool poisoned = bad || i2 < 0 || timed_out;
    if (poisoned) var = (double)__builtin_nanf("");
    const float fm = poisoned ? __builtin_nanf("") : (float)mu, fr = poisoned ? __builtin_nanf("") : (float)(1.0 / sqrt(var + (double)f.eps));
    s_par[ch] = fm; s_par[C + ch] = fr; s_par[2 * C + ch] = be;
    if (blockIdx.x == 0) {
      f.mean[ch] = fm; f.rstd[ch] = fr;
      if (f.thr) f.thr[ch] = f.relu ? fm - be / fr : -__builtin_inff();
      if (f.decay < 0.f) {
        if (f.mmean) f.mmean[ch] = fm;
        if (f.mvar) f.mvar[ch] = (float)var;
      } else {
        if (f.mmean) f.mmean[ch] -= (1.0f - f.decay) * (f.mmean[ch] - fm);
        if (f.mvar) f.mvar[ch] -= (1.0f - f.decay) * (f.mvar[ch] - (float)var);
      }
    }
  }
}

constexpr int kFaChunk = 5;
struct FaLane { int c, rpp, mfirst, mend; bool active; };
template <int NT>
__device__ __forceinline__ FaLane fa_lane(const int M, const int C, const int m0, const int nrows, const int c0, const int nch) {
  FaLane L;
  const int oct = nch >> 3;
  L.rpp = NT / oct;
  const int vc = threadIdx.x % oct, rr = threadIdx.x / oct;
  L.c = c0 + (vc << 3);
  L.active = rr < L.rpp && L.c < C;
  L.mend = (m0 + nrows < M) ? m0 + nrows : M;
  L.mfirst = m0 + rr;
  return L;
}
__device__ __forceinline__ void fa_load_chunk(const FaLane& L, const unsigned short* y, const int ldy, const int mbase, u32x4 (&v)[kFaChunk]) {
#pragma unroll
  for (int i = 0; i < kFaChunk; ++i) {
    const int m = mbase + i * L.rpp;
    v[i] = (L.active && m < L.mend) ? *reinterpret_cast<const u32x4*>(y + (size_t)m * ldy + L.c) : u32x4{0u, 0u, 0u, 0u};
  }
}
__device__ __forceinline__ void fa_finish_chunk(const FusedApply& f, const FaLane& L, const int C, const float* s_par, const int mbase,
                                                const u32x4 (&v)[kFaChunk]) {
  if (!L.active) return;
  float mu[8], rs[8], be[8];
#pragma unroll
  for (int j = 0; j < 8; ++j) { mu[j] = s_par[L.c + j]; rs[j] = s_par[C + L.c + j]; be[j] = s_par[2 * C + L.c + j]; }
#pragma unroll
  for (int i = 0; i < kFaChunk; ++i) {
    const int m = mbase + i * L.rpp;
    if (m < L.mend) {
      const unsigned w[4] = {v[i].x, v[i].y, v[i].z, v[i].w};
      unsigned q[4];
#pragma unroll
      for (int j = 0; j < 4; ++j) {
        const float lo = (bf_lo(w[j]) - mu[2 * j]) * rs[2 * j] + be[2 * j];
        const float hi = (bf_hi(w[j]) - mu[2 * j + 1]) * rs[2 * j + 1] + be[2 * j + 1];
        q[j] = f.relu ? pack2bf(relu_f(lo), relu_f(hi)) : pack2bf(lo, hi);
      }
      *reinterpret_cast<u32x4*>(f.a + (size_t)m * f.ld_a + L.c) = u32x4{q[0], q[1], q[2], q[3]};
    }
  }
}
template <int NT>
__device__ __forceinline__ void fused_apply_region(const FusedApply& f, const unsigned short* y, const int ldy, const int M, const int C,
                                                   const float* s_par, const int m0, const int nrows, const int c0, const int nch,
                                                   const int skip_chunks = 0) {
  const FaLane L = fa_lane<NT>(M, C, m0, nrows, c0, nch);
  for (int mb = L.mfirst + skip_chunks * kFaChunk * L.rpp; mb < L.mend; mb += kFaChunk * L.rpp) {
    u32x4 v[kFaChunk];
    fa_load_chunk(L, y, ldy, mb, v);
    fa_finish_chunk(f, L, C, s_par, mb, v);
  }
}

template <int NT>
__device__ __forceinline__ bool fused_grid_meet(const FusedApply& f, int* s_flag) {
  if (threadIdx.x == 0)
    *s_flag = (f.fault & kProbeNoWait) ? 0 : (grid_barrier_arrive_wait(f.bar, gridDim.x, blockIdx.x, f.spin_limit, f.fault & 1, f.step_poison) ? 1 : 0);
  __syncthreads();
  return *s_flag != 0;
}

template <int NT, class Regions>
__device__ __forceinline__ void fused_apply_tail(const ConvK& p, void* lds, const Regions& for_each_region) {
  const FusedApply& f = p.fa;
  float* s_par = reinterpret_cast<float*>(lds);
  int* s_flag = reinterpret_cast<int*>(s_par + 3 * p.C_out);
  const unsigned short* y = reinterpret_cast<const unsigned short*>(p.y);
  const int ldy = p.ldy, M = p.M, C = p.C_out;
  asm volatile("s_waitcnt vmcnt(0) lgkmcnt(0)" ::: "memory");
  __syncthreads();
  u32x4 v0[kFaChunk];
  FaLane L0;
  L0.active = false; L0.c = 0; L0.rpp = 1; L0.mfirst = 0; L0.mend = 0;
  int idx = 0;
  for_each_region([&](const int m0, const int nrows, const int c0, const int nch) {
    if (idx++ == 0) { L0 = fa_lane<NT>(M, C, m0, nrows, c0, nch); fa_load_chunk(L0, y, ldy, L0.mfirst, v0); }
  });
  const bool timed_out = fused_grid_meet<NT>(f, s_flag);
  fused_stats_to_lds<NT>(f, p.stats, p.stats_mod, p.stats_ld, C, s_par, timed_out);
  __syncthreads();
  if (f.fault & kProbeNoSweep) return;
  idx = 0;
  for_each_region([&](const int m0, const int nrows, const int c0, const int nch) {
    if (idx++ == 0) {
      fa_finish_chunk(f, L0, C, s_par, L0.mfirst, v0);
      fused_apply_region<NT>(f, y, ldy, M, C, s_par, m0, nrows, c0, nch, 1);
    } else {
      fused_apply_region<NT>(f, y, ldy, M, C, s_par, m0, nrows, c0, nch);
    }
  });
}


struct FbShared { FusedBwd f; int flag; int pad[3]; };

__device__ __forceinline__ FbShared* fused_bwd_stage(void* lds_area) {
  typedef const __attribute__((address_space(4))) unsigned* kernarg_words;
  const kernarg_words ka = (kernarg_words)__builtin_amdgcn_kernarg_segment_ptr() + offsetof(ConvK, fb) / 4;
  unsigned* dst = reinterpret_cast<unsigned*>(lds_area);
  for (int i = threadIdx.x; i < (int)(sizeof(FusedBwd) / 4); i += blockDim.x) dst[i] = ka[i];
  asm volatile("s_waitcnt vmcnt(0) lgkmcnt(0)" ::: "memory");
  __syncthreads();
  return reinterpret_cast<FbShared*>(lds_area);
}

__device__ __forceinline__ int fb_seg(const FusedBwd& f, const int c) { return (c >= f.cb[1]) + (c >= f.cb[2]) + (c >= f.cb[3]); }

typedef const __attribute__((address_space(1))) u32x4* g_u32x4_cptr;
typedef __attribute__((address_space(1))) u32x4* g_u32x4_ptr;
typedef const __attribute__((address_space(1))) f32x4u* g_f32x4_cptr;
typedef __attribute__((address_space(1))) float* g_f32_ptr;
template <class T> __device__ __forceinline__ unsigned long long gaddr(T* p) { return reinterpret_cast<unsigned long long>(p); }

struct FbLane {
  float mu[8], rs[8], be[8];
  unsigned long long y, dy, mean, rstd, beta;
  int ldy, lddy, relu;
  int c, rpp, mfirst, mend;
  bool active;
};
constexpr int kFbChunk = 4;

template <int NT>
__device__ __forceinline__ void fb_lane_geom(const FusedBwd& f, const int M, const int C, const int m0, const int nrows, const int c0, const int nch, FbLane& L) {
  const int oct = nch >> 3;
  L.rpp = NT / oct;
  const int vc = threadIdx.x % oct, rr = threadIdx.x / oct;
  L.c = c0 + (vc << 3);
  L.active = rr < L.rpp && L.c < C;
  L.mend = (m0 + nrows < M) ? m0 + nrows : M;
  L.mfirst = m0 + rr;
  const int cc = L.c < C ? L.c : 0;
  const int sg = fb_seg(f, cc), cr = cc - f.cb[sg];
  L.relu = f.relu[sg];
  L.ldy = f.ldy[sg]; L.lddy = f.lddy[sg];
  L.y = gaddr(f.y[sg] + cr); L.dy = gaddr(f.dy[sg] + cr);
  L.mean = gaddr(f.mean[sg] + cr); L.rstd = gaddr(f.rstd[sg] + cr);
  L.beta = L.relu ? gaddr(f.beta[sg] + cr) : L.mean;
}
__device__ __forceinline__ void fb_lane_params(FbLane& L) {
  const f32x4u a0 = *(g_f32x4_cptr)L.mean, a1 = *((g_f32x4_cptr)L.mean + 1);
  const f32x4u b0 = *(g_f32x4_cptr)L.rstd, b1 = *((g_f32x4_cptr)L.rstd + 1);
  const f32x4u c0 = *(g_f32x4_cptr)L.beta, c1 = *((g_f32x4_cptr)L.beta + 1);
  L.mu[0] = a0.x; L.mu[1] = a0.y; L.mu[2] = a0.z; L.mu[3] = a0.w; L.mu[4] = a1.x; L.mu[5] = a1.y; L.mu[6] = a1.z; L.mu[7] = a1.w;
  L.rs[0] = b0.x; L.rs[1] = b0.y; L.rs[2] = b0.z; L.rs[3] = b0.w; L.rs[4] = b1.x; L.rs[5] = b1.y; L.rs[6] = b1.z; L.rs[7] = b1.w;
  const float k = L.relu ? 1.f : 0.f;
  L.be[0] = c0.x * k; L.be[1] = c0.y * k; L.be[2] = c0.z * k; L.be[3] = c0.w * k; L.be[4] = c1.x * k; L.be[5] = c1.y * k; L.be[6] = c1.z * k; L.be[7] = c1.w * k;
}
__device__ __forceinline__ void fb_load_chunk(const FbLane& L, const unsigned short* da, const int ldg, const int mbase,
                                              u32x4 (&vg)[kFbChunk], u32x4 (&vy)[kFbChunk]) {
  const unsigned long long ga = gaddr(da) + 2ull * (unsigned)L.c;
#pragma unroll
  for (int i = 0; i < kFbChunk; ++i) {
    const int m = mbase + i * L.rpp;
    const bool ok = L.active && m < L.mend;
    const unsigned long long mm = ok ? (unsigned long long)m : 0ull;
    const u32x4 g = *(g_u32x4_cptr)(ga + 2ull * mm * (unsigned)ldg);
    const u32x4 y = *(g_u32x4_cptr)(L.y + 2ull * mm * (unsigned)L.ldy);
    vg[i] = ok ? g : u32x4{0u, 0u, 0u, 0u};
    vy[i] = y;
  }
}
__device__ __forceinline__ void fb_sums_chunk(const FbLane& L, const u32x4 (&vg)[kFbChunk], const u32x4 (&vy)[kFbChunk], float (&s1)[8], float (&s2)[8]) {
#pragma unroll
  for (int i = 0; i < kFbChunk; ++i) {
    const unsigned wg[4] = {vg[i].x, vg[i].y, vg[i].z, vg[i].w}, wy[4] = {vy[i].x, vy[i].y, vy[i].z, vy[i].w};
#pragma unroll
    for (int j = 0; j < 8; ++j) {
      const float g = (j & 1) ? bf_hi(wg[j >> 1]) : bf_lo(wg[j >> 1]);
      const float yy = (j & 1) ? bf_hi(wy[j >> 1]) : bf_lo(wy[j >> 1]);
      const float xh = (yy - L.mu[j]) * L.rs[j];
      const float gj = (!L.relu || xh + L.be[j] > 0.f) ? g : 0.f;
      s1[j] += gj;
      s2[j] += gj * xh;
    }
  }
}
__device__ __forceinline__ void fb_apply_chunk(const FusedBwd& f, const FbLane& L, const int C, const float* s_tot, const int mbase,
                                               const u32x4 (&vg)[kFbChunk], const u32x4 (&vy)[kFbChunk]) {
  if (!L.active) return;
  float m1[8], m2[8];
#pragma unroll
  for (int j = 0; j < 8; ++j) { m1[j] = s_tot[L.c + j]; m2[j] = s_tot[C + L.c + j]; }
#pragma unroll
  for (int i = 0; i < kFbChunk; ++i) {
    const int m = mbase + i * L.rpp;
    if (m < L.mend) {
      const unsigned wg[4] = {vg[i].x, vg[i].y, vg[i].z, vg[i].w}, wy[4] = {vy[i].x, vy[i].y, vy[i].z, vy[i].w};
      float o[8];
#pragma unroll
      for (int j = 0; j < 8; ++j) {
        const float g = (j & 1) ? bf_hi(wg[j >> 1]) : bf_lo(wg[j >> 1]);
        const float yy = (j & 1) ? bf_hi(wy[j >> 1]) : bf_lo(wy[j >> 1]);
        const float xh = (yy - L.mu[j]) * L.rs[j];
        const float gj = (!L.relu || xh + L.be[j] > 0.f) ? g : 0.f;
        o[j] = L.rs[j] * (gj - m1[j] - xh * m2[j]);
      }
      *(g_u32x4_ptr)(L.dy + 2ull * (unsigned long long)m * (unsigned)L.lddy) = u32x4{pack2bf(o[0], o[1]), pack2bf(o[2], o[3]), pack2bf(o[4], o[5]), pack2bf(o[6], o[7])};
    }
  }
}

template <int NT>
__device__ __forceinline__ void fb_reduce_region(const FusedBwd& f, const FbLane& L, const int C, const int c0, const int nch,
                                                 const float (&s1)[8], const float (&s2)[8], float* s_red, float* s_red2) {
  const int oct = nch >> 3, rpp = L.rpp, ncol = 16 * oct;
  const int vc = threadIdx.x % oct, rr = threadIdx.x / oct;
  if (rr < rpp) {
    float* o = s_red + ((size_t)rr * oct + vc) * 16;
#pragma unroll
    for (int j = 0; j < 8; ++j) { o[j] = s1[j]; o[8 + j] = s2[j]; }
  }
  __syncthreads();
  const int nsl = NT / ncol > 0 ? NT / ncol : 1;
  const int rps = (rpp + nsl - 1) / nsl;
  for (int e = threadIdx.x; e < nsl * ncol; e += NT) {
    const int col = e % ncol, sl = e / ncol;
    float t = 0.f;
    const int r1 = min(rpp, (sl + 1) * rps);
    for (int r = sl * rps; r < r1; ++r) t += s_red[(size_t)r * ncol + col];
    s_red2[e] = t;
  }
  __syncthreads();
  for (int e = threadIdx.x; e < ncol; e += NT) {
    float t = 0.f;
    for (int sl = 0; sl < nsl; ++sl) t += s_red2[sl * ncol + e];
    const int ch = c0 + ((e >> 4) << 3) + (e & 7);
    if (ch < C) {
      const int sg = fb_seg(f, ch);
      float* ap = f.acc[sg] + ((size_t)(blockIdx.x & (kFbSlots - 1)) * 2 + ((e >> 3) & 1)) * f.acc_ld[sg] + (ch - f.cb[sg]);
      __builtin_amdgcn_global_atomic_fadd_f32((g_f32_ptr)gaddr(ap), t);
    }
// ... 104 lines not shown
```

### multibox_amd/csrc/grid_barrier.h

```cpp
#pragma once
#include <hip/hip_runtime.h>

#ifndef MBX_GB_SLEEP
#define MBX_GB_SLEEP 8
#endif
constexpr int kGbSub = 16, kGbRel = 32, kGbLine = 32;
constexpr int kGbCtlWords = kGbLine * (2 + kGbSub + kGbRel);
constexpr int kFbSlots = 8;

__device__ __forceinline__ unsigned gb_ld(const unsigned* p) { return __hip_atomic_load(p, __ATOMIC_RELAXED, __HIP_MEMORY_SCOPE_AGENT); }
__device__ __forceinline__ long long gb_ld(const long long* p) { return __hip_atomic_load(p, __ATOMIC_RELAXED, __HIP_MEMORY_SCOPE_AGENT); }
__device__ __forceinline__ float gb_ld(const float* p) { return __hip_atomic_load(p, __ATOMIC_RELAXED, __HIP_MEMORY_SCOPE_AGENT); }

__device__ __forceinline__ bool grid_barrier_arrive_wait(unsigned* ctl, const unsigned G, const unsigned b, const unsigned spin_limit,
                                                         const int fault, float* step_poison) {
  const unsigned sub = b % kGbSub, n_sub = (G - sub + kGbSub - 1) / kGbSub, n_top = G < (unsigned)kGbSub ? G : (unsigned)kGbSub;
  bool timed_out = false;
  bool last = ((fault & 1) && b == 0) ? false : atomicAdd(ctl + kGbLine * (1 + sub), 1u) == n_sub - 1;
  if (last) last = atomicAdd(ctl + kGbLine * (1 + kGbSub), 1u) == n_top - 1;
  if (last) {
    for (int r = 0; r < kGbRel; ++r)
      __hip_atomic_store(ctl + kGbLine * (2 + kGbSub + r), 1u, __ATOMIC_RELAXED, __HIP_MEMORY_SCOPE_AGENT);
  } else {
    const unsigned* rel = ctl + kGbLine * (2 + kGbSub + b % kGbRel);
    unsigned spins = 0;
    while (gb_ld(rel) == 0u) {
      __builtin_amdgcn_s_sleep(MBX_GB_SLEEP);
      if (++spins > spin_limit) {
        ctl[1] = 1u;
        timed_out = true;
        if (step_poison) atomicAdd(step_poison, 1.0f);
        break;
      }
    }
  }
  if (b == 0) ctl[0] = G;
  return timed_out;
}

namespace mbx {

struct FusedApply {
  unsigned* bar;
  unsigned spin_limit; int fault;
  float* step_poison;
  unsigned short* a; int ld_a;
  const float* beta;
  float* mean; float* rstd; float* mmean; float* mvar; float* thr;
  int relu; float eps, decay; double inv_count;
};

struct FusedBwd {
  unsigned* bar;
  unsigned spin_limit; int fault;
  float* step_poison;
  int n;
  int cb[4];
  const unsigned short* y[4]; int ldy[4];
  unsigned short* dy[4]; int lddy[4];
  const float* mean[4]; const float* rstd[4]; const float* beta[4];
  float* dbeta[4];
  float* acc[4]; int acc_ld[4];
  int relu[4];
  float inv_M;
};

}
```

### multibox_amd/engine.py

```python
from __future__ import annotations

import ctypes as C
import math
import os
import re

import numpy as np
import torch

from . import _lib, ops
from .ops import View

BN_EPS = 0.001
STATS_ROWS = int(os.environ.get("MBX_STATS_ROWS", "8"))
WEIGHT_DECAY = 0.00004


def _same_pad(n, k, s):
    out = -(-n // s)
    total = max((out - 1) * s + k - n, 0)
    return out, total // 2


def _valid(n, k, s):
    return (n - k) // s + 1, 0


class ParamSpec:

    def __init__(self, scope, K, R, S, Cin, bn, bias):
        self.scope, self.K, self.R, self.S, self.Cin, self.bn, self.bias = scope, K, R, S, Cin, bn, bias


class ConvOp:

    def __init__(self, net, members, x: View, out: View, R, S, stride, pad_t, pad_l, kind, relu=True, skip=None,
                 rscale=0.0, trainable=True, need_dx=True, head=None):
        self.net, self.members, self.x, self.out = net, members, x, out
        self.R, self.S, self.stride, self.pad_t, self.pad_l = R, S, stride, pad_t, pad_l
        self.kind, self.relu, self.skip, self.rscale = kind, relu, skip, rscale
        self.trainable, self.need_dx, self.head = trainable, need_dx, head
        self.K = sum(m.K for m in members)
        self.Cin = x.C
        self.M = out.M
        self.name = members[0].scope if len(members) == 1 else "+".join(m.scope for m in members)
        self.group = None
        self.unit = None
        self.fused_pool = None
        self.relu_bits = None
        self.fdesc = None
        self.head_grad = None

    w_off = b_off = beta_off = dw_off = -1


class BnUnit:

    def __init__(self, members):
        self.members = list(members)
        self.lead = self.members[0]
        self.K = sum(m.K for m in members)
        self.koff, k = [], 0
        for m in members:
            self.koff.append(k)
            k += m.K
        self.y = self.dy = None
        self.fwd_desc, self.dgrad_desc = {}, {}
        self.pair_fwd = self.pair_bwd = False
        self.rows = [0] * len(members)
        self.stats_off = [0] * len(members)

    def chan_map(self, views):
        rel = [v.ch_off - ko for v, ko in zip(views, self.koff)]
        base = min(rel)
        m = _lib.ChanMap()
        m.n = len(self.members)
        for i, (ko, r) in enumerate(zip(self.koff, rel)):
            m.c_begin[i], m.offset[i] = ko, r - base
        return base, m

    def target(self, views):
        if len(views) == 1:
            return views[0].ptr, views[0].ld, None
        assert all(v.buf is views[0].buf and v.ld == views[0].ld for v in views)
        base, m = self.chan_map(views)
        return views[0].buf.data_ptr() + 2 * base, views[0].ld, m


def dgrad_probe(X):
    dd = ops.ConvDesc()
    dd.R, dd.S, dd.stride, dd.epilogue, dd.C_in, dd.C_out = X.R, X.S, 1, ops.EPI_STORE, X.K, X.Cin
    dd.N, dd.H_in, dd.W_in, dd.H_out, dd.W_out = X.x.N, X.out.H, X.out.W, X.x.H, X.x.W
    dd.rscale = X.rscale if X.kind == "residual" else 0.0
    return dd


def plan_consumer_fusion(convs, fwd, unit_ok, consumer_ok, align):
    is_conv = set(id(c) for c in convs)
    units = [op.unit for op in convs if op.kind == "bn" and op.trainable and op is op.unit.lead and op.unit.K <= 2048
             and unit_ok(op.unit)]

    def member_at(buf, c):
        for u in units:
            for m in u.members:
                if m.out.buf is buf and m.out.ch_off <= c < m.out.ch_off + m.K:
                    return m
        return None

    def readers(buf, lo, hi):
        r = [o for o in fwd if o.x.buf is buf and o.x.ch_off < hi and o.x.ch_off + o.x.C > lo]
        r += [o for o in fwd if id(o) in is_conv and o.skip is not None and o.skip.buf is buf and
              o.skip.ch_off < hi and o.skip.ch_off + o.skip.C > lo]
        return r

    def segments(X):
        segs, c, end = [], X.x.ch_off, X.x.ch_off + X.x.C
        while c < end:
            m = member_at(X.x.buf, c)
            if m is None:
                return None
            n = min(end, m.out.ch_off + m.K) - c
            segs.append((c - X.x.ch_off, m, c - m.out.ch_off, n))
            c += n
        if len(segs) > 4 or any(sg[0] % align for sg in segs):
            return None
        return segs

    eligible = set(id(u) for u in units)
    while True:
        conv_ok = {}
        for X in fwd:
            if id(X) not in is_conv or not X.need_dx or not X.trainable or X.stride != 1:
                continue
            segs = segments(X)
            if segs is None or any(id(sg[1].unit) not in eligible for sg in segs):
                continue
            if len(readers(X.x.buf, X.x.ch_off, X.x.ch_off + X.x.C)) != 1:
                continue
            if consumer_ok(X):
                conv_ok[id(X)] = (X, segs)
        drop = set()
        for u in units:
            if id(u) not in eligible:
                continue
            for m in u.members:
                rd = readers(m.out.buf, m.out.ch_off, m.out.ch_off + m.K)
                covered = sorted((max(o.x.ch_off, m.out.ch_off), min(o.x.ch_off + o.x.C, m.out.ch_off + m.K)) for o in rd)
                tiled = bool(covered) and covered[0][0] == m.out.ch_off and covered[-1][1] == m.out.ch_off + m.K and \
                    all(a[1] == b[0] for a, b in zip(covered, covered[1:]))
                if not tiled or any(id(o) not in conv_ok for o in rd):
                    drop.add(id(u))
        if not drop:
            return [u for u in units if id(u) in eligible], dict(conv_ok.values())
        eligible -= drop


class Net:
    def __init__(self, batch, input_size=299, k=5, mode="train", fine_tune=False, device="cuda", seed=2,
                 bn_decay=0.9997, repeats=(10, 20, 9), bn_max_workgroups=0, wgrad_overlap_cus=None):
        assert mode in ("train", "infer")
        self.repeats = tuple(repeats)
        self.B, self.S, self.k, self.mode, self.fine_tune, self.dev = batch, input_size, k, mode, fine_tune, device
        self.bn_decay = bn_decay
        self.tune_registry = []
        self.deterministic = bool(int(os.environ.get("MBX_DETERMINISTIC", "0")))
        self.no_onepass = self.deterministic or bool(int(os.environ.get("MBX_NO_BN_ONEPASS", "0")))
        self.atomic_stats = mode == "train" and not self.deterministic and os.environ.get("MBX_ATOMIC_STATS", "1") != "0"
        self.bw_stats = self.atomic_stats and os.environ.get("MBX_BW_STATS", "0") == "1"
        self.fuse_apply = self.atomic_stats and os.environ.get("MBX_FUSE_APPLY", "0") == "1"
        self.fused_apply_launches = 0
        self.fuse_bwd = (mode == "train" and not self.deterministic and not self.bw_stats and torch.device(device).type == "cuda"
                         and os.environ.get("MBX_FUSE_BWD", "0") == "1")
        self.fused_bwd_launches = self.fused_bwd_layers = 0
        self.relu_bits = mode == "train" and os.environ.get("MBX_RELU_BITS", "1") != "0"
        self.autotune = torch.device(device).type == "cuda" and bool(int(os.environ.get("MBX_AUTOTUNE", "1")))
        self.bn_max_wg = int(os.environ.get("MBX_BN_MAX_WG", "0")) or (bn_max_workgroups or 0)
        self.wgrad_overlap_cus = ops.wgrad_overlap_cus() if wgrad_overlap_cus is None else int(wgrad_overlap_cus)
        self.n_cus = torch.cuda.get_device_properties(device).multi_processor_count if torch.device(device).type == "cuda" else 256
        self.chain_cap = 0
        if self.wgrad_overlap_cus > 0 and mode == "train":
            self.wgrad_overlap_cus = min(self.wgrad_overlap_cus, self.n_cus // 2)
            self.chain_cap = min(self.bn_max_wg or self.n_cus, self.n_cus - self.wgrad_overlap_cus)
        self.cu_cap = 0
        self.defer_moving = False
        self.i5_counters = torch.zeros(8192, dtype=torch.int32, device=device)
        self._i5_used = 0
        self._probe_skip_apply = self._probe_skip_bn_bwd = False
        self.convs, self.fwd, self.bwd = [], [], []
        self._bn_group_requests, self.bn_groups = [], []
        self.grad_alias = {}
        self.written = set()
        self.heads = []
        self._bufs = []
        self._keep = []
        self._build()
        self._finalize(seed)

    def alloc(self, H, W, Cc, dtype=torch.bfloat16, zero=False):
        v = View.alloc(self.B, H, W, Cc, dtype=dtype, device=self.dev, zero=zero)
        self._bufs.append(v.buf)
        return v

    def grad_of(self, v: View) -> View:
        key = id(v.buf)
        if key not in self.grad_alias:
            g = torch.zeros_like(v.buf)
            self._bufs.append(g)
            self.grad_alias[key] = g
        return View(self.grad_alias[key], v.N, v.H, v.W, v.C, v.ld, v.ch_off, v.elem_size)

    def share_grad(self, v: View, like: View):
        self.grad_alias[id(v.buf)] = self.grad_of(like).buf

    def _training_bn(self, is_head):
        if self.mode == "infer":
            return False
        return is_head if self.fine_tune else True

    def conv(self, members, x, out, kh, kw, stride=1, padding="SAME", kind=None, relu=True, skip=None, rscale=0.0,
             is_head=False, need_dx=True, head=None):
        fh = _same_pad if padding == "SAME" else _valid
        Ho, pt = fh(x.H, kh, stride)
        Wo, pl = fh(x.W, kw, stride)
        assert (Ho, Wo) == (out.H, out.W), (members, Ho, Wo, out.H, out.W)
        if kind is None:
            kind = "bn" if self._training_bn(is_head) else "frozen"
        trainable = self.mode == "train" and (is_head or not self.fine_tune)
        specs = [ParamSpec(s, K, kh, kw, x.C, bn=kind in ("bn", "frozen"), bias=kind == "residual") for s, K in members]
        op = ConvOp(self, specs, x, out, kh, kw, stride, pt, pl, kind, relu, skip, rscale, trainable,
                    need_dx and trainable, head)
        op.is_head = is_head
        assert op.K == out.C or kind == "head", (op.name, op.K, out.C)
        self.convs.append(op)
        self.fwd.append(op)
        return op

    def group_bn(self, *members):
        if os.environ.get("MBX_BN_GROUPS", "1") != "0" and len(members) >= 2:
            self._bn_group_requests.append(members)

    def _build(self):
        B, S, k = self.B, self.S, self.k
        P = "InceptionResnetV2/"
        self.images = self.alloc(S, S, 8)
        s1, _ = _valid(S, 3, 2)
        a1 = self.alloc(s1, s1, 32)
        self.conv([(P + "Conv2d_1a_3x3", 32)], self.images, a1, 3, 3, 2, "VALID", need_dx=False)
        s2 = s1 - 2
        a2 = self.alloc(s2, s2, 32)
        self.conv([(P + "Conv2d_2a_3x3", 32)], a1, a2, 3, 3, 1, "VALID")
        a3 = self.alloc(s2, s2, 64)
        self.conv([(P + "Conv2d_2b_3x3", 64)], a2, a3, 3, 3, 1, "SAME")
        s3, _ = _valid(s2, 3, 2)
        p3 = self.alloc(s3, s3, 64)
        self.pool("max", a3, p3, 3, 2, scope=P + "MaxPool_3a_3x3")
        a4 = self.alloc(s3, s3, 80)
        self.conv([(P + "Conv2d_3b_1x1", 80)], p3, a4, 1, 1, 1, "VALID")
        s4 = s3 - 2
        a5 = self.alloc(s4, s4, 192)
        self.conv([(P + "Conv2d_4a_3x3", 192)], a4, a5, 3, 3, 1, "VALID")
        s5, _ = _valid(s4, 3, 2)
        t5 = self.alloc(s5, s5, 192)
        self.pool("max", a5, t5, 3, 2, scope=P + "MaxPool_5a_3x3")

        Q = P + "Mixed_5b/"
        z = self.alloc(s5, s5, 528)
        self.conv([(Q + "Branch_1/Conv2d_0a_1x1", 48), (Q + "Branch_2/Conv2d_0a_1x1", 64), (Q + "Branch_0/Conv2d_1x1", 96)],
                  t5, z.slice(0, 208), 1, 1)
        ga = self.conv([(Q + "Branch_1/Conv2d_0b_5x5", 64)], z.slice(0, 48), z.slice(208, 64), 5, 5)
        gb = self.conv([(Q + "Branch_2/Conv2d_0b_3x3", 96)], z.slice(48, 64), z.slice(432, 96), 3, 3)
        self.group_bn(ga, gb)
        self.conv([(Q + "Branch_2/Conv2d_0c_3x3", 96)], z.slice(432, 96), z.slice(272, 96), 3, 3)
        p5 = self.alloc(s5, s5, 192)
        self.pool("avg", t5, p5, 3, 1, pad=1, scope=Q + "Branch_3/AvgPool_0a_3x3")
        self.conv([(Q + "Branch_3/Conv2d_0b_1x1", 64)], p5, z.slice(368, 64), 1, 1)
        net = z.slice(112, 320)
        self.endpoints = {"MaxPool_5a_3x3": t5, "Mixed_5b": net}

        trunk0 = net
        zg = None
        for i in range(1, self.repeats[0] + 1):
            Q = P + "Repeat/block35_%d/" % i
            z = self.alloc(s5, s5, 240)
            if zg is None:
                zg = z
            else:
                self.share_grad(z, zg)
            self.conv([(Q + "Branch_1/Conv2d_0a_1x1", 32), (Q + "Branch_2/Conv2d_0a_1x1", 32), (Q + "Branch_0/Conv2d_1x1", 32)],
                      net, z.slice(0, 96), 1, 1)
            ga = self.conv([(Q + "Branch_1/Conv2d_0b_3x3", 32)], z.slice(0, 32), z.slice(96, 32), 3, 3)
            gb = self.conv([(Q + "Branch_2/Conv2d_0b_3x3", 48)], z.slice(32, 32), z.slice(192, 48), 3, 3)
            self.group_bn(ga, gb)
            self.conv([(Q + "Branch_2/Conv2d_0c_3x3", 64)], z.slice(192, 48), z.slice(128, 64), 3, 3)
            out = self.alloc(s5, s5, 320)
            self.residual(Q + "Conv2d_1x1", z.slice(64, 128), net, out, 0.17, True, trunk0)
            net = out

        Q = P + "Mixed_6a/"
        s6, _ = _valid(s5, 3, 2)
        o6 = self.alloc(s6, s6, 1088)
        self.conv([(Q + "Branch_0/Conv2d_1a_3x3", 384)], net, o6.slice(0, 384), 3, 3, 2, "VALID")
        t6a = self.alloc(s5, s5, 256)
        self.conv([(Q + "Branch_1/Conv2d_0a_1x1", 256)], net, t6a, 1, 1)
        t6b = self.alloc(s5, s5, 256)
        self.conv([(Q + "Branch_1/Conv2d_0b_3x3", 256)], t6a, t6b, 3, 3)
        self.conv([(Q + "Branch_1/Conv2d_1a_3x3", 384)], t6b, o6.slice(384, 384), 3, 3, 2, "VALID")
        self.pool("max", net, o6.slice(768, 320), 3, 2, scope=Q + "Branch_2/MaxPool_1a_3x3")
        self.endpoints["block35_10"] = net
        net = o6
        self.endpoints["Mixed_6a"] = net

        trunk0, zg = net, None
        for i in range(1, self.repeats[1] + 1):
            Q = P + "Repeat_1/block17_%d/" % i
            z = self.alloc(s6, s6, 672)
            if zg is None:
                zg = z
            else:
                self.share_grad(z, zg)
            self.conv([(Q + "Branch_1/Conv2d_0a_1x1", 128), (Q + "Branch_0/Conv2d_1x1", 192)], net, z.slice(0, 320), 1, 1)
            self.conv([(Q + "Branch_1/Conv2d_0b_1x7", 160)], z.slice(0, 128), z.slice(512, 160), 1, 7)
            self.conv([(Q + "Branch_1/Conv2d_0c_7x1", 192)], z.slice(512, 160), z.slice(320, 192), 7, 1)
            out = self.alloc(s6, s6, 1088)
# ... 253 lines not shown
        for op in self.convs:
            u = op.fb_unit
            if u is not None and op is u.lead:
                ws_floats = (ws_floats + 31) // 32 * 32
                op.fb_acc_off = ws_floats
                ws_floats += ops.BN_BWD_SLOTS * 2 * u.K
            if op.fb_segments is not None:
                ws_floats = (ws_floats + 31) // 32 * 32
                op.fb_bar_off = ws_floats
                ws_floats += ops.GRID_BARRIER_BYTES // 4
        ws_floats = (ws_floats + 31) // 32 * 32
        self.bn_ws = torch.zeros(max(ws_floats, 8), dtype=torch.float32, device=dev)
        assert self.bn_ws.data_ptr() % 128 == 0 or torch.device(dev).type != "cuda"
        n_ctr = self.i5_counters.numel()
        n_stats16 = (max(n_stats16, 4) + 31) // 32 * 32
        self._n_fwd_barriers = sum(1 for op in self.convs if op.kind == "bn") if self.fuse_apply else 0
        self._fwd_barriers_used = 0
        bar_words = ops.GRID_BARRIER_BYTES // 4
        self._fwd_clear = torch.zeros(n_ctr + n_stats16 + self._n_fwd_barriers * bar_words + 32, dtype=torch.int32, device=dev)
        self.i5_counters = self._fwd_clear[:n_ctr]
        self.stats16 = self._fwd_clear[n_ctr:n_ctr + n_stats16].view(torch.float32)
        b0 = n_ctr + n_stats16
        b0 += (-(self._fwd_clear.data_ptr() // 4 + b0)) % 32
        self._fwd_barrier_base = self._fwd_clear.data_ptr() + 4 * b0
        self.bn_thr = torch.zeros(max(self.nBt, 8), dtype=torch.float32, device=dev)
        self.bn_timeouts_total = torch.zeros((), dtype=torch.int64, device=dev)
        self.stats_scratch = torch.zeros(max(max_stats, 2), dtype=torch.float32, device=dev)
        self.bwd_scratch = torch.zeros(max(max_bwd, 2), dtype=torch.float32, device=dev)
        self.m12 = torch.zeros(2 * 2048, dtype=torch.float32, device=dev)
        self.reg_loss = torch.zeros(1, dtype=torch.float32, device=dev)

    def _plan_bw_stats(self):
        for op in self.convs:
            op.bw_unit, op.bw_segments = None, None
        if not self.bw_stats or torch.device(self.dev).type != "cuda":
            return

        def consumer_ok(X):
            dd = dgrad_probe(X)
            return not (ops.direct3_applies(dd) or ops.directw_applies(dd) or ops.resident_applies(dd))

        units, segs = plan_consumer_fusion(self.convs, self.fwd, lambda u: True, consumer_ok, align=32)
        for u in units:
            for m in u.members:
                m.bw_unit = u
        for X, sg in segs.items():
            X.bw_segments = sg

    def _plan_fused_bwd(self):
        for op in self.convs:
            op.fb_unit, op.fb_segments = None, None
        if not self.fuse_bwd:
            return
        pairs_ok = os.environ.get("MBX_FUSE_BWD_PAIRS", "1") != "0"
        only = re.compile(os.environ["MBX_FUSE_BWD_ONLY"]) if os.environ.get("MBX_FUSE_BWD_ONLY") else None
        max_rounds = int(os.environ.get("MBX_FUSE_BWD_MAX_ROUNDS", "1"))

        def consumer_ok(X):
            if X.x.img_stride != X.x.H * X.x.W * X.x.ld or X.Cin % 8 or (only is not None and not only.search(X.name)):
                return False
            if not pairs_ok and X.kind == "bn" and len(X.unit.members) == 2:
                return False
            dd = dgrad_probe(X)
            if ops.direct3_applies(dd):
                return False
            return ops.fused_tail_rounds(dd, self.n_cus) <= max_rounds

        units, segs = plan_consumer_fusion(self.convs, self.fwd, lambda u: all(m.fused_pool is None for m in u.members),
                                           consumer_ok, align=8)
        for u in units:
            for m in u.members:
                m.fb_unit = u
        for X, sg in segs.items():
            X.fb_segments = sg

    def _fb_table(self, X):
        t = ops.BnBwdFused()
        t.barrier = self.bn_ws.data_ptr() + 4 * X.fb_bar_off
        t.n = len(X.fb_segments)
        t.step_poison = self.step_ctl.data_ptr()
        for i, (c_rel, m, c_in, n) in enumerate(X.fb_segments):
            u = m.unit
            ko = m.y_view.ch_off
            assert m.y_view.ld == u.K and m.dy_view.ld == u.K and u.lead.fb_acc_off >= 0
            t.c_begin[i] = c_rel
            t.y[i], t.ld_y[i] = m.y_view.buf.data_ptr() + 2 * (ko + c_in), u.K
            t.dy[i], t.ld_dy[i] = m.dy_view.buf.data_ptr() + 2 * (ko + c_in), u.K
            t.mean[i] = self.bn_mean.data_ptr() + 4 * (m.beta_off + c_in)
            t.rstd[i] = self.bn_rstd.data_ptr() + 4 * (m.beta_off + c_in)
            t.beta[i] = self.Bt.data_ptr() + 4 * (m.beta_off + c_in)
            t.dbeta[i] = self.Btg.data_ptr() + 4 * (m.beta_off + c_in)
            t.acc[i], t.acc_ld[i] = self.bn_ws.data_ptr() + 4 * (u.lead.fb_acc_off + ko + c_in), u.K
            t.relu[i] = int(m.relu)
        self._keep.append(t)
        return t

    def _bw_table(self, X):
        t = _lib.BnBwdStats()
        t.n, t.rows_mod = len(X.bw_segments), STATS_ROWS
        for i, (c_rel, m, c_in, n) in enumerate(X.bw_segments):
            u = m.unit
            ko = m.y_view.ch_off
            t.c_begin[i] = c_rel
            t.y[i], t.ld_y[i] = m.y_view.buf.data_ptr() + 2 * (ko + c_in), u.K
            t.relu_thr[i] = self.bn_thr.data_ptr() + 4 * (m.beta_off + c_in)
            t.stats[i], t.stats_ld[i] = self.bn_ws.data_ptr() + 4 * (u.lead.bw_rows_off + 2 * (ko + c_in)), u.K
        self._keep.append(t)
        return t

    def _w(self, op):
        return self.Wb[op.w_off:]

    def _desc(self, op, y: View, **kw):
        return ops.make_desc(op.x, self._w(op), op.K, op.R, op.S, op.stride, op.pad_t, op.pad_l, y, **kw)

    def _sl(self, t, off, n):
        return t[off:off + n]

    def _tune(self, op, d, what):
        key = (what, op.x.N, op.x.H, op.x.W, op.x.C, op.K, op.R, op.S, op.stride, op.pad_t, op.pad_l, d.C_out, d.C_in,
               d.epilogue, bool(d.stats_partial), d.accumulate, bool(d.skip) or (bool(d.relu_bits) and d.epilogue == ops.EPI_STORE), d.relu)
        if d.relu_bits and d.epilogue == ops.EPI_RESIDUAL:
            key = key + ("bits",)
        self.tune_registry.append((repr(key), d, what))
        if self.autotune:
            ops.autotune(d, key)
            over = ops._TUNED.get(repr(key) + "#norule") if os.environ.get("MBX_NO_RULE_EXCEPTIONS") != "1" else None
            if over is not None:
                keep = d.tile_config
                d.tile_config = int(over)
                if _lib.lib().mbx_conv_supported(C.byref(d)) != 0:
                    d.tile_config, over = keep, None
            if os.environ.get("MBX_NO_I5") == "1" and d.tile_config > ops.I5_FLAG:
                d.tile_config = ops._TUNED.get(repr(key) + "#i3", 0)
            if d.tile_config > ops.I5_FLAG and os.environ.get("MBX_I5_STATIC") != "1":
                n = ops.I7_COUNTERS if d.tile_config == ops.I7_TILE_CONFIG else 1
                assert self._i5_used + n <= self.i5_counters.numel()
                d.work_counter = self.i5_counters.data_ptr() + 4 * self._i5_used
                self._i5_used += n
            if os.environ.get("MBX_NO_2STAGE") == "1":
                d.tile_config = {9: 7, 10: 2, 11: 5, 12: 2, 13: 8, 14: 1}.get(d.tile_config, d.tile_config)
            pair = (what == "fwd" and bool(d.stats_partial) and op.group is not None and len(op.group.members) == 2
                    and os.environ.get("MBX_CONV_PAIR", "1") != "0")
            rule = ops.launch_rule(d, pair) if over is None else None
            if rule is not None:
                d.tile_config, d.work_counter = rule[0], None
                _lib.check(_lib.lib().mbx_conv_supported(C.byref(d)), rule[1] + " " + op.name)
        return d

    def _build_forward_launches(self):
        L = []
        l = _lib.lib()
        st = lambda: torch.cuda.current_stream().cuda_stream
        for op in self.fwd:
            if isinstance(op, PoolOp):
                if not op.fused_fwd:
                    L.append(op.forward)
                continue
            if op.kind == "bn":
                L.append(self._bn_forward(op))
            elif op.kind == "frozen":
                d = self._tune(op, self._desc(op, op.out, epilogue=ops.EPI_AFFINE, relu=op.relu,
                                              scale=self._sl(self.bn_scale, op.beta_off, op.K),
                                              shift=self._sl(self.bn_shift, op.beta_off, op.K)), "fwd")
                L.append(lambda d=d, op=op: _lib.check(l.mbx_conv(C.byref(d), st()), op.name))
            elif op.kind == "residual":
                d = self._tune(op, self._desc(op, op.out, epilogue=ops.EPI_RESIDUAL, relu=op.relu,
                                              shift=self._sl(self.W, op.b_off, op.K), skip=op.skip, rscale=op.rscale,
                                              relu_bits=op.relu_bits), "fwd")
                L.append(lambda d=d, op=op: _lib.check(l.mbx_conv(C.byref(d), st()), op.name))
            elif op.kind == "head":
                d = self._desc(op, op.out, epilogue=ops.EPI_STORE_F32)
                L.append(lambda d=d, op=op: _lib.check(l.mbx_conv(C.byref(d), st()), op.name))
                if op is self.heads[-1]:
                    L.append(lambda: _lib.check(l.mbx_head_gather_all(self.head_table, len(self.heads), self.B, self.P,
                                                                      self.locs.data_ptr(), self.logits.data_ptr(), st()), "head_gather_all"))
        return L

    def _bn_forward(self, op):
        l = _lib.lib()
        st = lambda: torch.cuda.current_stream().cuda_stream
        cuda = torch.device(self.dev).type == "cuda"
        u = op.unit
        i, n, single = u.members.index(op), len(u.members), len(u.members) == 1
        fpool = op.fused_pool
        use16 = self.atomic_stats and fpool is None
        if use16:
            d = self._desc(op, op.y_view, stats=self.stats16[op.stats16_off:], stats_rows_mod=STATS_ROWS, stats_ld=0 if single else u.K)
        else:
            d = self._desc(op, op.y_view, stats=self.stats_scratch[op.stats_off:])
        d = self._tune(op, d, "fwd")
        S_ = ops.splitk_slices(d, self.n_cus) if single and cuda else 0
        if S_:
            d.tile_config = ops.SPLITK_FLAG + S_
            need = int(l.mbx_conv_splitk_workspace_bytes(C.byref(d)))
            ws = torch.empty(need // 4, dtype=torch.float32, device=self.dev)
            self._keep.append(ws)
            d.splitk_ws, d.splitk_ws_bytes = ws.data_ptr(), ws.numel() * 4
            _lib.check(l.mbx_conv_supported(C.byref(d)), "split-K " + op.name)
        rows = u.rows[i] = ops.conv_stats_rows(d)
        assert use16 or i + 1 == n or rows * op.K * 2 <= u.stats_off[i + 1] - u.stats_off[i]
        u.fwd_desc[i] = d
        if i + 1 < n:
            return lambda: None if u.pair_fwd else _lib.check(l.mbx_conv(C.byref(d), st()), op.name)
        if n == 2 and cuda and os.environ.get("MBX_CONV_PAIR", "1") != "0":
            u.pair_fwd = l.mbx_conv_pair(C.byref(u.fwd_desc[0]), C.byref(d), st()) == 0
        K, M, out = u.K, op.M, op.out
        mean, rstd, mm, mv, var, beta, thr = (self._sl(t, u.lead.beta_off, K) for t in
                                              (self.bn_mean, self.bn_rstd, self.MM, self.MV, self.bn_var, self.Bt, self.bn_thr))
        s16 = self.stats16[u.stats16_base:]
        a_ptr, a_ld, amap = u.target([m.out for m in u.members])
        amap = None if amap is None else C.byref(amap)
        parts = (C.c_void_p * n)(*[self.stats_scratch.data_ptr() + 4 * o for o in u.stats_off])
        rows_a, cs_a = (C.c_int32 * n)(*u.rows), (C.c_int32 * n)(*[m.K for m in u.members])
        if fpool is not None:
            fpool.fused_fwd = True
        fd = ba = None
        if single and use16 and self.fuse_apply and not S_ and cuda and out.img_stride == out.H * out.W * out.ld \
                and (not os.environ.get("MBX_FUSE_APPLY_ONLY") or re.search(os.environ["MBX_FUSE_APPLY_ONLY"], op.name)):
            ba = ops.BnApplyDesc()
            ba.barrier = self._fwd_barrier_base + ops.GRID_BARRIER_BYTES * self._fwd_barriers_used
            ba.a, ba.ld_a, ba.beta, ba.mean, ba.rstd = out.ptr, out.ld, beta.data_ptr(), mean.data_ptr(), rstd.data_ptr()
            ba.relu_thr, ba.relu, ba.eps, ba.step_poison = thr.data_ptr(), int(op.relu), BN_EPS, self.step_ctl.data_ptr()
            fd = ops.ConvDesc.from_buffer_copy(d)
            fd.bn_apply = C.addressof(ba)
            fd.work_counter = None
            if l.mbx_conv_supported(C.byref(fd)) == 0:
                assert self._fwd_barriers_used < self._n_fwd_barriers
                self._fwd_barriers_used += 1
                self.fused_apply_launches += 1
            else:
                fd = ba = None

        def run():
            s = st()
            mm_, mv_, decay = (None, var, -1.0) if self.defer_moving else (mm, mv, self.bn_decay)
            if fd is not None and not self.no_onepass:
                ba.moving_mean, ba.moving_var, ba.decay = ops._p(mm_), ops._p(mv_), decay
                fd.max_workgroups = self.cu_cap or self.bn_max_wg
                _lib.check(l.mbx_conv(C.byref(fd), s), op.name + " + bn apply")
                return
            if u.pair_fwd:
                _lib.check(l.mbx_conv_pair(C.byref(u.fwd_desc[0]), C.byref(d), s), "pair " + op.name)
            else:
                _lib.check(l.mbx_conv(C.byref(d), s), op.name)
            totals = (mean.data_ptr(), rstd.data_ptr(), ops._p(mm_), ops._p(mv_))
            if use16:
                _lib.check(l.mbx_bn_apply_fused_mapped(s16.data_ptr(), STATS_ROWS, M, BN_EPS, decay, u.y.data_ptr(), M, K,
                                                       beta.data_ptr(), int(op.relu), a_ptr, a_ld, amap, *totals,
                                                       thr.data_ptr(), s), "bn_apply_fused_mapped")
            elif not single:
                _lib.check(l.mbx_bn_finalize_parts(parts, rows_a, cs_a, n, M, BN_EPS, decay, *totals, s), "bn_finalize_parts")
                _lib.check(l.mbx_bn_apply_mapped(u.y.data_ptr(), M, K, mean.data_ptr(), rstd.data_ptr(), beta.data_ptr(),
                                                 int(op.relu), a_ptr, a_ld, amap, s), "bn_apply_mapped")
            elif fpool is not None:
                po = fpool.out
                _lib.check(l.mbx_bn_finalize(self.stats_scratch.data_ptr(), rows, K, M, BN_EPS, decay, *totals, s), "bn_finalize")
                _lib.check(l.mbx_bn_apply_maxpool(u.y.data_ptr(), out.N, out.H, out.W, K, mean.data_ptr(), rstd.data_ptr(),
                                                  beta.data_ptr(), int(op.relu), po.ptr, po.img_stride, po.ld, po.H, po.W,
                                                  fpool.argmax.data_ptr(), s), "bn_apply_maxpool")
            elif self._probe_skip_apply and ("/block" in op.name or "/Block8" in op.name):
                _lib.check(l.mbx_bn_finalize(self.stats_scratch.data_ptr(), rows, K, M, BN_EPS, decay, *totals, s), "fin")
            else:
                _lib.check(l.mbx_bn_apply_fused(self.stats_scratch.data_ptr(), rows, M, BN_EPS, decay, u.y.data_ptr(), M, K,
                                                beta.data_ptr(), int(op.relu), a_ptr, a_ld, *totals, s), "bn_apply_fused")
        return run

    def _gview(self, v: View) -> View:
        return self.grad_of(v)

    def _claim(self, g: View):
        key = (id(g.buf), g.ch_off, g.C)
        if key in self.written:
            return 1, None
        self.written.add(key)
        src = self.pending_acc.pop(key, None)
        return (1, src) if src is not None else (0, None)

    def _make_head_table(self):
        arr = (_lib.Head * len(self.heads))()
        for j, op in enumerate(self.heads):
            cells, kk, off = op.head
            if self.mode == "train":
                op.head_grad = View(torch.zeros((op.M, self.head_ld), dtype=torch.bfloat16, device=self.dev),
                                    op.out.N, op.out.H, op.out.W, self.head_ld)
                self._bufs.append(op.head_grad.buf)
            arr[j].h, arr[j].ld_h = op.out.buf.data_ptr(), self.head_ld
            arr[j].g, arr[j].ld_g = (op.head_grad.buf.data_ptr() if op.head_grad is not None else None), self.head_ld
            arr[j].cells, arr[j].k, arr[j].off = cells, kk, off
        self.head_table = arr

    def _build_backward(self):
        self._make_head_table()
        if self.mode != "train":
            self.fwd_launches = self._build_forward_launches()
            self.bwd_launches = []
            self.bwd_jobs = []
            return
        l = _lib.lib()
        st = lambda: torch.cuda.current_stream().cuda_stream
        entries, d_off, blocks = [], 0, 0
        for op in self.convs:
            if op.need_dx:
                kpad = (op.K + 7) // 8 * 8
                e = _lib.FilterEntry(op.w_off, d_off, op.K, op.R, op.S, op.Cin, kpad, blocks)
                op.dgrad_off, op.kpad = d_off, kpad
                n = op.Cin * op.R * op.S * kpad
                d_off += (n + 7) // 8 * 8
                blocks += op.R * op.S * ((op.Cin + 31) // 32) * ((kpad + 63) // 64)
                entries.append(e)
        self.Wd = torch.zeros(max(d_off, 8), dtype=torch.bfloat16, device=self.dev)
        arr = (_lib.FilterEntry * len(entries))(*entries)
        raw = np.frombuffer(C.string_at(C.addressof(arr), C.sizeof(arr)), dtype=np.uint8).copy()
        self.filter_table = torch.from_numpy(raw).to(self.dev)
        self.filter_blocks, self.filter_entries = blocks, len(entries)

        mask_of = {}
        fused_mask = set()
        for r in self.convs:
            if r.kind == "residual" and r.relu and r.trainable:
                for c in self.fwd:
                    if isinstance(c, ConvOp) and c.x.buf is r.out.buf:
                        if c.need_dx and c.x.ch_off == r.out.ch_off and c.x.C == r.out.C:
                            mask_of[id(c)] = r
                            fused_mask.add(id(r))
                        break
                    if isinstance(c, PoolOp) and c.x.buf is r.out.buf:
                        break
        self.pending_acc = {}
        L = []
        self.bwd_ops = []
        self.bwd_jobs = []
        for op in reversed(self.fwd):
            if isinstance(op, PoolOp):
                if op.needs_backward():
                    prod = self._pool_producer(op)
                    if prod is not None:
                        prod.fused_pool = op
                        continue
                    gx = self._gview(op.x)
                    acc, src = self._claim(gx)
                    assert src is None, "a pooling layer cannot be the first writer of a residual block's input gradient"
                    L.append(op.make_backward(self._gview(op.out), gx, acc))
                    self.bwd_ops.append(op)
                    self.bwd_jobs.append(None)
                continue
            if not op.trainable:
                continue
            K, M = op.K, op.M
            dw = self._sl(self.Wg, op.w_off, K * op.R * op.S * op.Cin)
            if op.kind == "head":
                cells, kk, off = op.head
                g = op.head_grad
                dyv, scale, db = g, 1.0, None
                pre = None
                if op is self.heads[-1]:
                    pre = lambda s: _lib.check(l.mbx_head_scatter_all(self.d_locs.data_ptr(), self.d_logits.data_ptr(), self.head_table,
                                                                      len(self.heads), self.B, self.P, s), "head_scatter_all")
            elif op.kind == "residual":
                gout = self._gview(op.out)
                gs = self._gview(op.skip)
                self.pending_acc[(id(gs.buf), gs.ch_off, gs.C)] = gout
                zb = id(self.grad_of(op.x).buf)
                self.written = {k for k in self.written if k[0] != zb}
                dyv, scale, db = gout, op.rscale, self._sl(self.Wg, op.b_off, K)
                if op.relu and id(op) not in fused_mask:
                    pre = lambda s, gout=gout, op=op: _lib.check(
                        l.mbx_relu_mask(gout.ptr, gout.ld, op.out.ptr, op.out.ld, op.M, op.K, s), "relu_mask")
                else:
                    pre = None
            else:
                dyv, scale, db = op.dy_view, 1.0, None
                pre = self._bn_backward(op)
            ddesc = fdesc = None
            if op.need_dx:
                gx = self._gview(op.x)
                acc, acc_src = self._claim(gx)
                dyin = View(dyv.buf, dyv.N, dyv.H, dyv.W, op.kpad, dyv.ld, dyv.ch_off, 2)
                mr = mask_of.get(id(op))
                ddesc = ops.make_desc(dyin, self.Wd[op.dgrad_off:], op.Cin, op.R, op.S, op.stride,
                                      op.R - 1 - op.pad_t, op.S - 1 - op.pad_l, gx, transposed=1, accumulate=acc,
                                      rscale=(scale if scale != 1.0 else 0.0), skip=(mr.out if mr is not None else None),
                                      acc_src=acc_src)
                if mr is not None and self.relu_bits and op.Cin % 8 == 0:
                    bits = torch.zeros((op.x.N * op.x.H * op.x.W, (op.Cin + 31) // 32 * 4), dtype=torch.uint8, device=self.dev)
                    alt = ops.make_desc(dyin, self.Wd[op.dgrad_off:], op.Cin, op.R, op.S, op.stride,
                                        op.R - 1 - op.pad_t, op.S - 1 - op.pad_l, gx, transposed=1, accumulate=acc,
                                        rscale=(scale if scale != 1.0 else 0.0), acc_src=acc_src, relu_bits=bits)
                    if torch.device(self.dev).type != "cuda" or l.mbx_conv_supported(C.byref(alt)) == 0:
                        ddesc, mr.relu_bits = alt, bits
                self._tune(op, ddesc, "dgrad")
                if op.fb_segments is not None:
                    assert acc == 0 and acc_src is None and mr is None, op.name
                    fdesc = ops.ConvDesc.from_buffer_copy(ddesc)
                    fdesc.bn_bwd = C.addressof(self._fb_table(op))
                    fdesc.work_counter = None
                    if not (ops.I5_FLAG < fdesc.tile_config <= ops.I5_FLAG + 7 or fdesc.tile_config in (ops.DIRECTW_TILE_CONFIG, ops.RESIDENT_TILE_CONFIG)):
                        fdesc.tile_config = ops.i5_tile_for(op.x.M, op.Cin, self.n_cus)
                    if l.mbx_conv_supported(C.byref(fdesc)) != 0:
                        fdesc.tile_config = ops.i5_tile_for(op.x.M, op.Cin, self.n_cus)
# ... 280 lines not shown
```

### multibox_amd/ops.py

```python
from __future__ import annotations

import ctypes as C
import os

import torch

from . import _lib

EPI_STORE, EPI_AFFINE, EPI_RESIDUAL, EPI_STORE_F32 = 0, 1, 2, 3


class ConvDesc(C.Structure):
    _fields_ = [
        ("x", C.c_void_p), ("x_img_stride", C.c_int64), ("ldx", C.c_int32),
        ("N", C.c_int32), ("H_in", C.c_int32), ("W_in", C.c_int32), ("C_in", C.c_int32),
        ("w", C.c_void_p), ("C_out", C.c_int32), ("R", C.c_int32), ("S", C.c_int32),
        ("stride", C.c_int32), ("transposed", C.c_int32), ("pad_t", C.c_int32), ("pad_l", C.c_int32),
        ("H_out", C.c_int32), ("W_out", C.c_int32),
        ("y", C.c_void_p), ("y_img_stride", C.c_int64), ("ldy", C.c_int32),
        ("epilogue", C.c_int32), ("relu", C.c_int32), ("accumulate", C.c_int32),
        ("scale", C.c_void_p), ("shift", C.c_void_p),
        ("skip", C.c_void_p), ("skip_img_stride", C.c_int64), ("ld_skip", C.c_int32), ("rscale", C.c_float),
        ("stats_partial", C.c_void_p),
        ("tile_config", C.c_int32),
        ("acc_src", C.c_void_p), ("acc_img_stride", C.c_int64), ("ld_acc", C.c_int32),
        ("work_counter", C.c_void_p),
        ("max_workgroups", C.c_int32),
        ("splitk_ws", C.c_void_p), ("splitk_ws_bytes", C.c_int64),
        ("stats_rows_mod", C.c_int32), ("stats_ld", C.c_int32),
        ("bn_bwd_stats", C.c_void_p),
        ("relu_bits", C.c_void_p), ("ld_bits", C.c_int32),
        ("bn_apply", C.c_void_p),
        ("bn_bwd", C.c_void_p),
    ]


class BnApplyDesc(C.Structure):
    _fields_ = [("barrier", C.c_void_p), ("a", C.c_void_p), ("ld_a", C.c_int32), ("beta", C.c_void_p), ("mean", C.c_void_p),
                ("rstd", C.c_void_p), ("moving_mean", C.c_void_p), ("moving_var", C.c_void_p), ("relu_thr", C.c_void_p),
                ("relu", C.c_int32), ("eps", C.c_float), ("decay", C.c_float), ("step_poison", C.c_void_p)]


class BnBwdFused(C.Structure):
    _fields_ = [("barrier", C.c_void_p), ("n", C.c_int32), ("c_begin", C.c_int32 * 4), ("y", C.c_void_p * 4), ("ld_y", C.c_int32 * 4),
                ("dy", C.c_void_p * 4), ("ld_dy", C.c_int32 * 4), ("mean", C.c_void_p * 4), ("rstd", C.c_void_p * 4),
                ("beta", C.c_void_p * 4), ("dbeta", C.c_void_p * 4), ("acc", C.c_void_p * 4), ("acc_ld", C.c_int32 * 4),
                ("relu", C.c_int32 * 4), ("step_poison", C.c_void_p)]


GRID_BARRIER_BYTES = 6400
BN_BWD_SLOTS = 8


def i5_tile_for(M, C_out, n_cus=256):
    best, best_key = None, None
    for i, (bm, bn) in enumerate(I5_TILES):
        if (bm, bn) == (128, 192):
            continue
        t = -(-M // bm) * -(-C_out // bn)
        key = (0, -t, 0) if t <= n_cus else (1, -(-t // n_cus), -(-t // n_cus) * bm * bn)
        if best_key is None or key < best_key:
            best, best_key = I5_FLAG + 1 + i, key
    return best


def fused_tail_rounds(desc, n_cus=256):
    M = desc.N * desc.H_out * desc.W_out
    if resident_applies(desc, min_images=1):
        return -(-desc.N * 4 // n_cus)
    if directw_applies(desc):
        th = max(1, 256 // desc.W_out)
        return -(-desc.N * -(-desc.H_out // th) // n_cus)
    return min(-(-(-(-M // bm) * -(-desc.C_out // bn)) // n_cus) for bm, bn in I5_TILES if (bm, bn) != (128, 192))


class WgradJob(C.Structure):
    _fields_ = [("desc", ConvDesc), ("dy", C.c_void_p), ("dy_img_stride", C.c_int64), ("ld_dy", C.c_int32),
                ("scale", C.c_float), ("dw", C.c_void_p), ("db", C.c_void_p)]


class WgradPlanInfo(C.Structure):
    _fields_ = [("n_layers", C.c_int32), ("n_items", C.c_int32), ("layers_off", C.c_int64), ("items_off", C.c_int64),
                ("queues_off", C.c_int64), ("heads_off", C.c_int64), ("flops", C.c_double), ("tally_off", C.c_int64)]


class View:
    __slots__ = ("buf", "N", "H", "W", "C", "ld", "ch_off", "elem_size")

    def __init__(self, buf, N, H, W, C, ld=None, ch_off=0, elem_size=2):
        self.buf, self.N, self.H, self.W, self.C = buf, N, H, W, C
        self.ld = C if ld is None else ld
        self.ch_off, self.elem_size = ch_off, elem_size
        assert buf.numel() * buf.element_size() >= N * H * W * self.ld * elem_size, "view larger than its buffer"

    @property
    def ptr(self):
        return self.buf.data_ptr() + self.ch_off * self.elem_size

    @property
    def img_stride(self):
        return self.H * self.W * self.ld

    @property
    def M(self):
        return self.N * self.H * self.W

    def slice(self, off, C):
        assert off + C <= self.C
        return View(self.buf, self.N, self.H, self.W, C, self.ld, self.ch_off + off, self.elem_size)

    def tensor(self):
        dt = self.buf.dtype
        flat = self.buf.reshape(-1)[: self.N * self.H * self.W * self.ld].reshape(self.N, self.H, self.W, self.ld)
        return flat[..., self.ch_off:self.ch_off + self.C]

    @staticmethod
    def alloc(N, H, W, C, ld=None, dtype=torch.bfloat16, device="cuda", zero=False):
        ld = C if ld is None else ld
        f = torch.zeros if zero else torch.empty
        buf = f((N, H, W, ld), dtype=dtype, device=device)
        if not zero and os.environ.get("MBX_POISON"):
            buf.fill_(float("nan"))
        return View(buf, N, H, W, C, ld, 0, torch.empty((), dtype=dtype).element_size())


def _stream():
    return torch.cuda.current_stream().cuda_stream


def _p(t):
    return None if t is None else t.data_ptr()


def make_desc(x: View, w, C_out, R, S, stride, pad_t, pad_l, y: View, transposed=0, epilogue=EPI_STORE, relu=0,
              accumulate=0, scale=None, shift=None, skip: View = None, rscale=0.0, stats=None, acc_src: View = None,
              stats_rows_mod=0, stats_ld=0, relu_bits=None, ld_bits=0):
    d = ConvDesc()
    d.x, d.x_img_stride, d.ldx = x.ptr, x.img_stride, x.ld
    d.N, d.H_in, d.W_in, d.C_in = x.N, x.H, x.W, x.C
    d.w, d.C_out, d.R, d.S = (w.data_ptr() if w is not None else None), C_out, R, S
    d.stride, d.transposed, d.pad_t, d.pad_l = stride, transposed, pad_t, pad_l
    d.H_out, d.W_out = y.H, y.W
    d.y, d.y_img_stride, d.ldy = y.ptr, y.img_stride, y.ld
    d.epilogue, d.relu, d.accumulate = epilogue, int(relu), int(accumulate)
    d.scale, d.shift = _p(scale), _p(shift)
    if skip is not None:
        d.skip, d.skip_img_stride, d.ld_skip = skip.ptr, skip.img_stride, skip.ld
    d.rscale = float(rscale)
    d.stats_partial = _p(stats)
    d.stats_rows_mod, d.stats_ld = int(stats_rows_mod), int(stats_ld)
    if acc_src is not None:
        d.acc_src, d.acc_img_stride, d.ld_acc = acc_src.ptr, acc_src.img_stride, acc_src.ld
    if relu_bits is not None:
        d.relu_bits, d.ld_bits = relu_bits.data_ptr(), int(ld_bits if ld_bits else relu_bits.shape[-1])
    return d


def conv(desc: ConvDesc):
    _lib.check(_lib.lib().mbx_conv(C.byref(desc), _stream()), "mbx_conv")


def conv_stats_rows(desc: ConvDesc):
    r = _lib.lib().mbx_conv_stats_rows(C.byref(desc))
    if r < 0:
        _lib.check(r, "mbx_conv_stats_rows")
    return r


def conv_wgrad(desc: ConvDesc, dy: View, dw, db=None):
    _lib.check(_lib.lib().mbx_conv_wgrad(C.byref(desc), dy.ptr, dy.img_stride, dy.ld, dw.data_ptr(), _p(db), _stream()),
               "mbx_conv_wgrad")


WG_OVERLAP_DEFAULT = 0


def wgrad_overlap_cus():
    return max(0, int(os.environ.get("MBX_WG_OVERLAP", WG_OVERLAP_DEFAULT)))


N_TILE_CONFIGS = 14
I5_FLAG = 32
I5_TILE_CONFIGS = (33, 34, 35, 36, 37, 38, 39)
I5_TILES = ((128, 64), (128, 128), (192, 128), (256, 128), (256, 64), (128, 192), (128, 256))
I7_TILE_CONFIG = 65
I7_COUNTERS = 32
SPLITK_FLAG = 128
DIRECT3_TILE_CONFIG = 96


def direct3_applies(desc: ConvDesc, min_pixels=300000):
    if os.environ.get("MBX_DIRECT3", "1") == "0":
        return False
    if desc.R != 3 or desc.S != 3 or desc.epilogue not in (EPI_STORE, EPI_AFFINE) or desc.accumulate or desc.skip \
            or desc.rscale != 0.0 or (desc.epilogue == EPI_AFFINE and desc.stats_partial) or desc.bn_bwd_stats:
        return False
    if desc.stride == 2 and not desc.transposed and desc.C_in == 8 and desc.C_out <= 32 and desc.C_out % 8 == 0:
        pass
    elif desc.stride != 1 or desc.C_in not in (32, 64) or desc.C_out > 64 or desc.C_out % 8 or (desc.C_in == 64 and desc.C_out > 48):
        return False
    if -(-desc.W_out // 32) * 32 > 1.15 * desc.W_out:
        return False
    return desc.N * desc.H_out * desc.W_out >= int(os.environ.get("MBX_DIRECT3_MIN_PIXELS", min_pixels))


DIRECTW_TILE_CONFIG = 97


def directw_applies(desc: ConvDesc, min_pixels=60000):
    if os.environ.get("MBX_DIRECTW", "1") == "0":
        return False
    if desc.R != 3 or desc.S != 3 or desc.stride != 1 or desc.epilogue not in (EPI_STORE, EPI_AFFINE) or desc.accumulate or desc.skip \
            or desc.rscale != 0.0 or (desc.epilogue == EPI_AFFINE and desc.stats_partial) or desc.bn_bwd_stats:
        return False
    if desc.C_in not in (32, 48, 64) or desc.C_out > 64 or desc.C_out % 8 or (desc.C_in == 64 and desc.C_out > 48):
        return False
    if not (8 <= desc.W_out <= 64) or desc.W_in > desc.W_out + 2:
        return False
    return desc.N * desc.H_out * desc.W_out >= int(os.environ.get("MBX_DIRECTW_MIN_PIXELS", min_pixels))


RESIDENT_TILE_CONFIG = 98


def resident_applies(desc: ConvDesc, min_images=32):
    if os.environ.get("MBX_RESIDENT", "1") == "0":
        return False
    if desc.R * desc.S not in (3, 7) or min(desc.R, desc.S) != 1 or desc.stride != 1 or desc.epilogue not in (EPI_STORE, EPI_AFFINE) \
            or desc.accumulate or desc.skip or desc.rscale != 0.0 or (desc.epilogue == EPI_AFFINE and desc.stats_partial) \
            or desc.bn_bwd_stats or desc.relu_bits:
        return False
    if desc.H_in != desc.H_out or desc.W_in != desc.W_out or not (64 <= desc.H_out * desc.W_out <= 289):
        return False
    if desc.N < int(os.environ.get("MBX_RESIDENT_MIN_IMAGES", min_images)):
        return False
    if not desc.x or not desc.w or not desc.y:
        hw = desc.H_out * desc.W_out
        if desc.C_out % 8:
            return False
        if desc.R * desc.S == 3:
            return hw == 64 and desc.C_in in (192, 224, 256)
        return 65 <= hw <= 289 and desc.C_in in (128, 160, 192)
    keep = desc.tile_config
    desc.tile_config = RESIDENT_TILE_CONFIG
    ok = _lib.lib().mbx_conv_supported(C.byref(desc)) == 0
    desc.tile_config = keep
    return ok


PWRES_DEFAULT = "2"
PWRES_TILE_CONFIG = 99


def pwres_applies(desc: ConvDesc, min_pixels=4096):
    mode = os.environ.get("MBX_PWRES", PWRES_DEFAULT)
    if mode == "0":
        return False
    if desc.R != 1 or desc.S != 1 or desc.stride != 1 or desc.pad_t or desc.pad_l or desc.stats_partial or desc.bn_bwd_stats:
        return False
    if desc.C_in not in (96, 128, 320, 384, 448) or desc.C_out < 256 or desc.C_out % 8:
        return False
    res = desc.epilogue == EPI_RESIDUAL
    accm = desc.epilogue == EPI_STORE and desc.relu_bits and not desc.skip
    if not (res or accm) or (mode == "2" and not accm):
        return False
    return desc.N * desc.H_out * desc.W_out >= int(os.environ.get("MBX_PWRES_MIN_PIXELS", min_pixels))


def launch_rule(desc: ConvDesc, pair=False):
    if direct3_applies(desc):
        return DIRECT3_TILE_CONFIG, "direct 3x3"
    if directw_applies(desc) and not pair:
        return DIRECTW_TILE_CONFIG, "direct 3x3 (whole-width)"
    if pwres_applies(desc):
        return PWRES_TILE_CONFIG, "pixel-resident 1x1"
    if resident_applies(desc):
        return RESIDENT_TILE_CONFIG, "resident image"
    return None


def splitk_slices(desc: ConvDesc, n_cus=256):
    if os.environ.get("MBX_SPLITK", "1") == "0" or desc.transposed or desc.epilogue != EPI_STORE or desc.accumulate or desc.skip:
        return 0
    ktot = desc.R * desc.S * desc.C_in
    M = desc.N * desc.H_out * desc.W_out
    tiles = ((M + 127) // 128) * ((desc.C_out + 63) // 64)
    if ktot < 8192 or tiles > 96:
        return 0
    s = int(os.environ.get("MBX_SPLITK_SLICES", "0")) or max(2, min(16, (2 * n_cus) // tiles))
    return min(s, 32)
_TUNED = {}
TUNE_STATS = {"hits": 0, "remeasured": 0, "rejected": 0}
_TUNE_FILE = os.path.join(os.path.dirname(os.path.abspath(__file__)), "tune_cache.json")


def _load_tune_cache():
    if os.environ.get("MBX_TUNE_CACHE", "1") != "0" and os.path.exists(_TUNE_FILE):
        try:
            import json
            with open(_TUNE_FILE) as f:
                _TUNED.update({k: int(v) for k, v in json.load(f).items()})
        except (OSError, ValueError):
            pass


def save_tune_cache(path=None):
    import json
    with open(path or _TUNE_FILE, "w") as f:
        json.dump(dict(sorted(_TUNED.items())), f, indent=0)


_load_tune_cache()


def autotune(desc: ConvDesc, key, candidates=None, iters=10):
    key = repr(key)
    if key in _TUNED:
        desc.tile_config = _TUNED[key]
        if _lib.lib().mbx_conv_supported(C.byref(desc)) == 0:
            TUNE_STATS["hits"] += 1
            return desc.tile_config
        del _TUNED[key]
        TUNE_STATS["rejected"] += 1
    TUNE_STATS["remeasured"] += 1
    if candidates is None:
        candidates = (0, 2, 4, 5, 6, 9, 10, 12, 13, 14)
        if os.environ.get("MBX_AUTOTUNE_SET") == "all":
            candidates = tuple(range(0, N_TILE_CONFIGS + 1))
    l = _lib.lib()
    best, best_t = 0, float("inf")
    s = _stream()
    iters = int(os.environ.get("MBX_TUNE_ITERS", iters))
    for cfg in candidates:
        desc.tile_config = cfg
        if l.mbx_conv(C.byref(desc), s) != 0:
            continue
        e0, e1 = torch.cuda.Event(enable_timing=True), torch.cuda.Event(enable_timing=True)
        e0.record()
        for _ in range(iters):
            l.mbx_conv(C.byref(desc), s)
        e1.record()
        e1.synchronize()
        t = e0.elapsed_time(e1)
        if t < best_t * 0.97 or (cfg == 0 and t < best_t):
            best, best_t = cfg, t
    desc.tile_config = best
    _TUNED[key] = best
    return best


def autotune_wgrad(desc: ConvDesc, dy: View, scale, dw, db, key, candidates=(0, 2, 3, 4, 7, 8, 9, 10), iters=10):
    key = repr(key)
    if key in _TUNED:
        desc.tile_config = _TUNED[key]
        return desc.tile_config
    l = _lib.lib()
    s = _stream()
    best, best_t = 0, float("inf")
    iters = int(os.environ.get("MBX_TUNE_ITERS", iters))
    if os.environ.get("MBX_AUTOTUNE_WG"):
        candidates = tuple(int(v) for v in os.environ["MBX_AUTOTUNE_WG"].split(","))
    args = (dy.ptr, dy.img_stride, dy.ld, float(scale), dw.data_ptr(), _p(db), s)
    for cfg in candidates:
        desc.tile_config = cfg
        if l.mbx_conv_wgrad_scaled(C.byref(desc), *args) != 0:
            continue
        e0, e1 = torch.cuda.Event(enable_timing=True), torch.cuda.Event(enable_timing=True)
        e0.record()
        for _ in range(iters):
            l.mbx_conv_wgrad_scaled(C.byref(desc), *args)
        e1.record()
        e1.synchronize()
        t = e0.elapsed_time(e1)
        if t < best_t * 0.97 or (cfg == 0 and t < best_t):
            best, best_t = cfg, t
    desc.tile_config = best
    _TUNED[key] = best
    return best


class WgradGroup:

    def __init__(self, jobs, deterministic=False, device="cuda"):
        l = _lib.lib()
        self.n = len(jobs)
        arr = (WgradJob * self.n)(*jobs)
        flags = (1 if deterministic else 0) | (2 if os.environ.get("MBX_WGRAD_SCATTER") == "1" else 0)
        nbytes = l.mbx_wgrad_plan_bytes(arr, self.n, flags)
        assert nbytes > 0
        host = (C.c_uint8 * nbytes)()
        self.info = WgradPlanInfo()
        _lib.check(l.mbx_wgrad_plan(arr, self.n, flags, host, nbytes, C.byref(self.info)), "mbx_wgrad_plan")
        import numpy as np
        self.host_image = np.frombuffer(host, dtype=np.uint8).copy()
        self.image = torch.from_numpy(self.host_image).to(device)
        self.flops = float(self.info.flops)

    def launch(self, max_workgroups=0):
        _lib.check(_lib.lib().mbx_conv_wgrad_grouped_capped(self.image.data_ptr(), C.byref(self.info), int(max_workgroups),
                                                            _stream()), "mbx_conv_wgrad_grouped")
# ... 13 lines not shown
```

Before: 4372 images/sec.

## Fuse producer batch-norm apply into resident conv input staging

```diff
diff --git a/include/mbx.h b/include/mbx.h
--- a/include/mbx.h
+++ b/include/mbx.h
@@ -185,6 +185,16 @@
   int32_t relu[4];
   float* step_poison;
 } mbx_bn_bwd_fused;
+
+typedef struct {
+  const void* stats; int32_t rows;
+  void* a; int32_t ld_a;
+  const float* beta;
+  float* mean; float* rstd;
+  float* moving_mean; float* moving_var;
+  float* relu_thr;
+  int32_t relu; float eps, decay;
+} mbx_bn_input_desc;
 
 typedef struct {
   const void* x; int64_t x_img_stride; int32_t ldx;
@@ -206,6 +216,7 @@
   void* relu_bits; int32_t ld_bits;
   const mbx_bn_apply_desc* bn_apply;
   const mbx_bn_bwd_fused* bn_bwd;
+  const mbx_bn_input_desc* bn_input;
 } mbx_conv_desc;
 #define MBX_CONV_TILE_CONFIGS 14
 #define MBX_TILE_I5_BASE 32
diff --git a/multibox_amd/csrc/conv.hip b/multibox_amd/csrc/conv.hip
--- a/multibox_amd/csrc/conv.hip
+++ b/multibox_amd/csrc/conv.hip
@@ -570,6 +570,23 @@
     k.fa.relu = b->relu; k.fa.eps = b->eps; k.fa.decay = b->decay;
     k.fa.inv_count = 1.0 / (double)((long long)d->N * d->H_out * d->W_out);
   }
+  k.fin = nullptr;
+  FusedInput fin{};
+  if (d->bn_input) {
+    const mbx_bn_input_desc* b = d->bn_input;
+    if (!b->stats || !b->a || !b->beta || !b->mean || !b->rstd || b->rows < 1 || (reinterpret_cast<uintptr_t>(b->stats) & 15) ||
+        (reinterpret_cast<uintptr_t>(b->a) & 15) || b->ld_a % 8 || b->ld_a < d->C_in)
+      return MBX_ERR_INVALID_ARG;
+    if (b->rows > 16 || d->tile_config != kResidentCfg || d->transposed || d->stride != 1 || !d->stats_partial || d->bn_apply || d->bn_bwd ||
+        d->epilogue != MBX_EPI_STORE || d->rscale != 0.f)
+      return MBX_ERR_UNSUPPORTED;
+    fin.stats = reinterpret_cast<const float*>(b->stats); fin.rows = b->rows;
+    fin.f.a = reinterpret_cast<unsigned short*>(b->a); fin.f.ld_a = b->ld_a; fin.f.beta = b->beta;
+    fin.f.mean = b->mean; fin.f.rstd = b->rstd; fin.f.mmean = b->moving_mean; fin.f.mvar = b->moving_var; fin.f.thr = b->relu_thr;
+    fin.f.relu = b->relu; fin.f.eps = b->eps; fin.f.decay = b->decay;
+    fin.f.inv_count = 1.0 / (double)((long long)d->N * d->H_in * d->W_in);
+    k.fin = &fin;
+  }
   k.bw_n = 0; k.bw_mod = 1;
   for (int i = 0; i < 4; ++i) { k.bw_cb[i] = 1 << 30; k.bw_ldy[i] = 0; k.bw_sld[i] = 0; k.bw_y[i] = nullptr; k.bw_thr[i] = nullptr; k.bw_stats[i] = nullptr; }
   if (d->bn_bwd_stats) {
diff --git a/multibox_amd/csrc/conv_common.h b/multibox_amd/csrc/conv_common.h
--- a/multibox_amd/csrc/conv_common.h
+++ b/multibox_amd/csrc/conv_common.h
@@ -36,6 +36,7 @@
   int* work_counter;
   int max_wg;
   int dry;
+  const FusedInput* fin;
   int ksplit, kps; long long y_split_stride;
 #ifdef MBX_I5_STAMPS
   unsigned long long* stamps;
@@ -63,6 +64,7 @@
 using mbx::ConvK;
 using mbx::FusedApply;
 using mbx::FusedBwd;
+using mbx::FusedInput;
 
 typedef __attribute__((ext_vector_type(8))) __bf16 bf16x8;
 typedef __attribute__((ext_vector_type(4))) float f32x4;
diff --git a/multibox_amd/csrc/convr.hip b/multibox_amd/csrc/convr.hip
--- a/multibox_amd/csrc/convr.hip
+++ b/multibox_amd/csrc/convr.hip
@@ -18,7 +18,21 @@
   int per;
   int npi;
   int dh[9], dw[9], dd[9];
+  FusedInput fi;
 };
+
+__device__ __forceinline__ u32x4 lds_rd16(const int addr) {
+  u32x4 v;
+  asm volatile("ds_read_b128 %0, %1" : "=v"(v) : "v"(addr) : "memory");
+  return v;
+}
+__device__ __forceinline__ void lds_wr16(const int addr, const u32x4 v) { asm volatile("ds_write_b128 %0, %1" ::"v"(addr), "v"(v) : "memory"); }
+__device__ __forceinline__ void lds_wait4(u32x4& a, u32x4& b, u32x4& c, u32x4& d) {
+  asm volatile("s_waitcnt lgkmcnt(0)" : "+v"(a), "+v"(b), "+v"(c), "+v"(d)::"memory");
+}
+__device__ __forceinline__ void lds_wait6(u32x4& a, u32x4& b, u32x4& c, u32x4& d, u32x4& e, u32x4& f) {
+  asm volatile("s_waitcnt lgkmcnt(0)" : "+v"(a), "+v"(b), "+v"(c), "+v"(d), "+v"(e), "+v"(f)::"memory");
+}
 
 template <int C8>
 __device__ __forceinline__ int rkey(int r) {
@@ -67,16 +81,17 @@
   }
 }
 
-template <int C8, int NB, int RS, int MI>
+template <int C8, int NB, int RS, int MI, int IBN = 0>
 struct ResG {
   static constexpr int HWMAX = 16 * kRCW * MI;
+  static constexpr int PAR_CH = IBN ? (6 * C8 + 15) / 16 * 16 : 0;
   static constexpr int KC = C8 / 4;
   static constexpr int SLOT_CH = NB * 16 * C8;
   static constexpr int PT = (SLOT_CH + 64 * kRLW - 1) / (64 * kRLW);
   static constexpr int SLOTP = PT * kRLW * 64;
   static constexpr int RED_CH = kRCW * NB * 16 * 2 * 4 / 16;
   static constexpr int img_ch(int hw) { return ((hw + 1) * C8 + 63) / 64 * 64; }
-  static constexpr int lds_bytes(int hw, int d) { return (RED_CH + d * SLOTP + img_ch(hw)) * 16; }
+  static constexpr int lds_bytes(int hw, int d) { return (RED_CH + PAR_CH + d * SLOTP + img_ch(hw)) * 16; }
   static constexpr int depth(int hw) {
     int d = RS;
     while (d > 2 && lds_bytes(hw, d) > 160 * 1024) --d;
@@ -84,16 +99,19 @@
   }
 };
 
-template <int C8, int NB, int RS, int MI, int HWC, int EV>
+template <int C8, int NB, int RS, int MI, int HWC, int EV, int IBN = 0>
 __global__ void __launch_bounds__(kRThreads)
 conv_resident_kernel(const ConvK p, const ResK q) {
-  using G = ResG<C8, NB, RS, MI>;
+  using G = ResG<C8, NB, RS, MI, IBN>;
+  static_assert(!IBN || EV == 1, "input batch norm: the forward training-mode launch");
+  static_assert(!IBN || 8 * C8 <= 64 * kRCW, "the input's channels are finalised by the multiplying waves, a thread each");
   constexpr int KC = G::KC, PT = G::PT, SLOTP = G::SLOTP, D = G::depth(HWC), DD = D < RS ? D : RS;
   constexpr int GR = D >= RS ? (RS < 4 ? RS : 4) : (D / 2 > 0 ? D / 2 : 1), G0 = GR < RS ? GR : RS;
   static_assert(D >= RS || D >= 2 * GR || GR == 1, "two groups in the ring");
   extern __shared__ __attribute__((aligned(16))) u32x4 smem[];
   float* const red = reinterpret_cast<float*>(smem);
-  u32x4* const ring = smem + G::RED_CH;
+  float* const s_par = reinterpret_cast<float*>(smem + G::RED_CH);
+  u32x4* const ring = smem + G::RED_CH + G::PAR_CH;
   u32x4* const img = ring + D * SLOTP;
 
   const int tid = threadIdx.x, lane = tid & 63;
@@ -110,6 +128,46 @@
       const int pix = ci / C8, cs = ci - pix * C8;
       const int c = cs ^ rkey<C8>(pix);
       glds16(xr, img + i * 64, pix < q.HW ? (xo + pix * p.ldx + c * 8) * 2 : (int)kOOB);
+    }
+  };
+
+  constexpr int PL = kRThreads / C8;
+  auto ibn_sweep = [&](const int im, int th, auto norm, const bool to_a) {
+    constexpr bool NORM = decltype(norm)::value;
+    asm volatile("" : "+v"(th));
+    const int c8 = th % C8, pl = th / C8;
+    float mu[8], rs[8], be[8];
+    if constexpr (NORM) {
+      const int par = lds_addr(s_par) + 32 * c8;
+      u32x4 m0 = lds_rd16(par), m1 = lds_rd16(par + 16), r0 = lds_rd16(par + 32 * C8), r1 = lds_rd16(par + 32 * C8 + 16);
+      u32x4 b0 = lds_rd16(par + 64 * C8), b1 = lds_rd16(par + 64 * C8 + 16);
+      lds_wait6(m0, m1, r0, r1, b0, b1);
+      const unsigned wm[8] = {m0.x, m0.y, m0.z, m0.w, m1.x, m1.y, m1.z, m1.w}, wr_[8] = {r0.x, r0.y, r0.z, r0.w, r1.x, r1.y, r1.z, r1.w};
+      const unsigned wb[8] = {b0.x, b0.y, b0.z, b0.w, b1.x, b1.y, b1.z, b1.w};
+#pragma unroll
+      for (int j = 0; j < 8; ++j) { mu[j] = __uint_as_float(wm[j]); rs[j] = __uint_as_float(wr_[j]); be[j] = __uint_as_float(wb[j]); }
+    }
+    const int img0 = lds_addr(img), relu = q.fi.f.relu, ld_a = q.fi.f.ld_a;
+    unsigned short* const a0 = q.fi.f.a + ((size_t)im * q.HW) * ld_a + 8 * c8;
+    for (int p0 = pl < PL ? pl : q.HW; p0 < q.HW; p0 += 4 * PL) {
+      u32x4 v[4];
+      int ad[4];
+#pragma unroll
+      for (int i = 0; i < 4; ++i) {
+        const int pix = p0 + i * PL < q.HW ? p0 + i * PL : p0;
+        ad[i] = img0 + 16 * (pix * C8 + (c8 ^ rkey<C8>(pix)));
+        v[i] = lds_rd16(ad[i]);
+      }
+      lds_wait4(v[0], v[1], v[2], v[3]);
+#pragma unroll
+      for (int i = 0; i < 4; ++i) {
+        const int pix = p0 + i * PL;
+        if (pix < q.HW) {
+          u32x4 w = v[i];
+          if constexpr (NORM) { w = fa_norm8(v[i], mu, rs, be, relu); lds_wr16(ad[i], w); }
+          if (to_a) *reinterpret_cast<u32x4*>(a0 + (size_t)pix * ld_a) = w;
+        }
+      }
     }
   };
 
@@ -144,6 +202,7 @@
           glds16(wr, dst + i * (kRLW * 64), (wv[i] && cb + rowch[i] < ce) ? wbase + wo[i] + tap * (8 * C8) * 2 : (int)kOOB);
       };
       auto slot_of = [&](const int rel) { return D == RS ? rel % RS : (base + rel) % D; };
+      const bool staged = t == t0 || im != im_in;
       if (t == t0) {
         issue_image(im);
 #pragma unroll
@@ -158,6 +217,12 @@
       im_in = im;
       lds_readback_wait(lds_readback_issue(ring + slot_of(G0 - 1) * SLOTP + (PT - 1) * (kRLW * 64) + lw * 64 + lane));
       raw_barrier();
+      if constexpr (IBN) {
+        if (staged) {
+          ibn_sweep(im, tid, std::true_type(), false);
+          lds_barrier();
+        }
+      }
 #pragma unroll
       for (int g0 = 0; g0 < RS; g0 += GR) {
         const int e = g0 + GR < RS ? g0 + GR : RS;
@@ -177,7 +242,7 @@
     }
   } else {
   const __amdgpu_buffer_rsrc_t yr = make_rsrc(p.y, p.y_bytes);
-  constexpr int RING_OFF0 = G::RED_CH * 16, IMG_OFF0 = RING_OFF0 + D * SLOTP * 16;
+  constexpr int RING_OFF0 = (G::RED_CH + G::PAR_CH) * 16, IMG_OFF0 = RING_OFF0 + D * SLOTP * 16;
   const int RING_OFF = RING_OFF0 + lds_addr(smem), IMG_OFF = IMG_OFF0 + lds_addr(smem);
   static_assert(RING_OFF0 % 256 == 0 && (SLOTP * 16) % 256 == 0, "the XOR-ed address bits of a row must be clear in the region offsets");
   int EA[NB];
@@ -217,6 +282,9 @@
     im_in = im;
     MBXR_STAMP(0);
     if (newim) issue_image(im);
+    if constexpr (IBN) {
+      if (t == first * q.per) fused_stats_to_lds<kRThreads, 8>(q.fi.f, q.fi.stats, q.fi.rows, 8 * C8, 8 * C8, s_par, false, first == 0);
+    }
     DirAffine<NB> af;
     direct_affine_load<EV, NB>(p, cb, ce, fch, af);
     if constexpr (EALL) {
@@ -230,6 +298,13 @@
       lds_readback_wait(lds_readback_issue(img + lane));
     }
     raw_barrier();
+    if constexpr (IBN) {
+      if (newim) {
+        ibn_sweep(im, tid, std::true_type(), g == 0);
+        lds_barrier();
+        if (g == 0) ibn_sweep(im, tid + kRThreads / 2, std::false_type(), true);
+      }
+    }
     MBXR_STAMP(1);
 #pragma unroll
     for (int a = 0; a < NB; ++a) asm volatile("" : "+v"(EA[a]));
@@ -588,6 +663,24 @@
   return launch_by_ev(k, q, grid, kRThreads, lds, s, [](auto ev) { return conv_resident_kernel<C8, NB, RS, MI, HWC, decltype(ev)::value>; });
 }
 
+template <int C8, int NB, int RS, int MI, int HWC>
+int launch_resident_ibn(const ConvK& k, const ResK& q, int grid, hipStream_t s) {
+  using G = ResG<C8, NB, RS, MI, 1>;
+  constexpr int lds = G::lds_bytes(HWC, G::depth(HWC));
+  static_assert(lds <= 160 * 1024, "LDS");
+  static_assert(G::depth(HWC) == ResG<C8, NB, RS, MI>::depth(HWC), "the parameter area leaves the ring its depth");
+  static_assert((G::RED_CH + G::PAR_CH) % 16 == 0, "the ring starts at a multiple of 256 bytes");
+  static_assert(HWC <= G::HWMAX && kRThreads / C8 <= 64, "pixel slots; a sweep step of the pass stays inside the smallest image");
+  static bool attr = false;
+  if (!attr) {
+    (void)hipFuncSetAttribute(reinterpret_cast<const void*>(conv_resident_kernel<C8, NB, RS, MI, HWC, 1, 1>), hipFuncAttributeMaxDynamicSharedMemorySize, lds);
+    attr = true;
+  }
+  hipLaunchKernelGGL((conv_resident_kernel<C8, NB, RS, MI, HWC, 1, 1>), dim3(grid), dim3(kRThreads), lds, s, k, q);
+  MBX_LAUNCH_CHECK();
+  return MBX_OK;
+}
+
 inline void resident_groups(int C_out, int& NG, int& CPT, int& NB) {
   NG = 4;
   CPT = ((C_out + NG * 8 - 1) / (NG * 8)) * 8;
@@ -618,6 +711,15 @@
   if (k.max_wg > 0 && grid > k.max_wg) grid = k.max_wg;
   q.per = (q.ntiles + grid - 1) / grid;
   grid = (q.ntiles + q.per - 1) / q.per;
+  q.fi = FusedInput{};
+  if (k.fin) {
+    if (k.epi != MBX_EPI_STORE || !k.stats || k.fa.bar || k.fb.bar) return MBX_ERR_UNSUPPORTED;
+    q.fi = *k.fin;
+    const bool b17 = C8 == 20 && NB == 3 && RS == 7 && q.HW > 64, b8 = C8 == 28 && NB == 4 && RS == 3 && q.HW == 64;
+    if (!b17 && !b8) return MBX_ERR_UNSUPPORTED;
+    if (k.dry) return MBX_OK;
+    return b17 ? launch_resident_ibn<20, 3, 7, 5, 289>(k, q, grid, s) : launch_resident_ibn<28, 4, 3, 1, 64>(k, q, grid, s);
+  }
 #define MBX_RES(C8_, NB_, RS_, MI_, HWC_)                                                                \
   if (C8 == C8_ && NB == NB_ && RS == RS_ && q.HW <= HWC_ && (HWC_ > 64 || q.HW == 64)) {                 \
     if (k.dry) return MBX_OK;                                                                            \
diff --git a/multibox_amd/csrc/fused_bn.h b/multibox_amd/csrc/fused_bn.h
--- a/multibox_amd/csrc/fused_bn.h
+++ b/multibox_amd/csrc/fused_bn.h
@@ -15,22 +15,26 @@
 }
 constexpr int kProbeNoWait = 16, kProbeNoTotals = 32, kProbeNoSweep = 64, kProbeNoSums = 128;
 
-template <int NT>
+template <int NT, int RB = 16>
 __device__ __forceinline__ void fused_stats_to_lds(const FusedApply& f, const float* stats, const int rows, const int ld, const int C,
-                                                   float* s_par, const bool timed_out) {
+                                                   float* s_par, const bool timed_out, const bool publish) {
   const __amdgpu_buffer_rsrc_t sr = make_rsrc(stats, (f.fault & kProbeNoTotals) ? 0u : (unsigned)(rows * ld * 16));
   for (int ch = threadIdx.x; ch < C; ch += NT) {
-    u32x4 v[16];
-#pragma unroll
-    for (int r = 0; r < 16; ++r) v[r] = ld16_agent(sr, r < rows ? (unsigned)((r * ld + ch) * 16) : kOOB);
     const float be = f.beta[ch];
     long long i1 = 0, i2 = 0;
     bool bad = false;
 #pragma unroll
-    for (int r = 0; r < 16; ++r) {
-      const long long v1 = (long long)(((unsigned long long)v[r].y << 32) | v[r].x), v2 = (long long)(((unsigned long long)v[r].w << 32) | v[r].z);
-      i1 += v1; i2 += v2;
-      bad |= v2 < 0;
+    for (int r0 = 0; r0 < 16; r0 += RB) {
+      if (r0 && r0 >= rows) break;
+      u32x4 v[RB];
+#pragma unroll
+      for (int r = 0; r < RB; ++r) v[r] = ld16_agent(sr, r0 + r < rows ? (unsigned)(((r0 + r) * ld + ch) * 16) : kOOB);
+#pragma unroll
+      for (int r = 0; r < RB; ++r) {
+        const long long v1 = (long long)(((unsigned long long)v[r].y << 32) | v[r].x), v2 = (long long)(((unsigned long long)v[r].w << 32) | v[r].z);
+        i1 += v1; i2 += v2;
+        bad |= v2 < 0;
+      }
     }
     const double s1 = (double)i1 * (1.0 / 1048576.0), s2 = (double)i2 * (1.0 / 1048576.0);
     const double mu = s1 * f.inv_count;
@@ -40,7 +44,7 @@
     if (poisoned) var = (double)__builtin_nanf("");
     const float fm = poisoned ? __builtin_nanf("") : (float)mu, fr = poisoned ? __builtin_nanf("") : (float)(1.0 / sqrt(var + (double)f.eps));
     s_par[ch] = fm; s_par[C + ch] = fr; s_par[2 * C + ch] = be;
-    if (blockIdx.x == 0) {
+    if (publish) {
       f.mean[ch] = fm; f.rstd[ch] = fr;
       if (f.thr) f.thr[ch] = f.relu ? fm - be / fr : -__builtin_inff();
       if (f.decay < 0.f) {
@@ -75,6 +79,17 @@
     v[i] = (L.active && m < L.mend) ? *reinterpret_cast<const u32x4*>(y + (size_t)m * ldy + L.c) : u32x4{0u, 0u, 0u, 0u};
   }
 }
+__device__ __forceinline__ u32x4 fa_norm8(const u32x4 v, const float (&mu)[8], const float (&rs)[8], const float (&be)[8], const int relu) {
+  const unsigned w[4] = {v.x, v.y, v.z, v.w};
+  unsigned q[4];
+#pragma unroll
+  for (int j = 0; j < 4; ++j) {
+    const float lo = (bf_lo(w[j]) - mu[2 * j]) * rs[2 * j] + be[2 * j];
+    const float hi = (bf_hi(w[j]) - mu[2 * j + 1]) * rs[2 * j + 1] + be[2 * j + 1];
+    q[j] = relu ? pack2bf(relu_f(lo), relu_f(hi)) : pack2bf(lo, hi);
+  }
+  return u32x4{q[0], q[1], q[2], q[3]};
+}
 __device__ __forceinline__ void fa_finish_chunk(const FusedApply& f, const FaLane& L, const int C, const float* s_par, const int mbase,
                                                 const u32x4 (&v)[kFaChunk]) {
   if (!L.active) return;
@@ -84,17 +99,7 @@
 #pragma unroll
   for (int i = 0; i < kFaChunk; ++i) {
     const int m = mbase + i * L.rpp;
-    if (m < L.mend) {
-      const unsigned w[4] = {v[i].x, v[i].y, v[i].z, v[i].w};
-      unsigned q[4];
-#pragma unroll
-      for (int j = 0; j < 4; ++j) {
-        const float lo = (bf_lo(w[j]) - mu[2 * j]) * rs[2 * j] + be[2 * j];
-        const float hi = (bf_hi(w[j]) - mu[2 * j + 1]) * rs[2 * j + 1] + be[2 * j + 1];
-        q[j] = f.relu ? pack2bf(relu_f(lo), relu_f(hi)) : pack2bf(lo, hi);
-      }
-      *reinterpret_cast<u32x4*>(f.a + (size_t)m * f.ld_a + L.c) = u32x4{q[0], q[1], q[2], q[3]};
-    }
+    if (m < L.mend) *reinterpret_cast<u32x4*>(f.a + (size_t)m * f.ld_a + L.c) = fa_norm8(v[i], mu, rs, be, f.relu);
   }
 }
 template <int NT>
@@ -134,7 +139,7 @@
     if (idx++ == 0) { L0 = fa_lane<NT>(M, C, m0, nrows, c0, nch); fa_load_chunk(L0, y, ldy, L0.mfirst, v0); }
   });
   const bool timed_out = fused_grid_meet<NT>(f, s_flag);
-  fused_stats_to_lds<NT>(f, p.stats, p.stats_mod, p.stats_ld, C, s_par, timed_out);
+  fused_stats_to_lds<NT>(f, p.stats, p.stats_mod, p.stats_ld, C, s_par, timed_out, blockIdx.x == 0);
   __syncthreads();
   if (f.fault & kProbeNoSweep) return;
   idx = 0;
diff --git a/multibox_amd/csrc/grid_barrier.h b/multibox_amd/csrc/grid_barrier.h
--- a/multibox_amd/csrc/grid_barrier.h
+++ b/multibox_amd/csrc/grid_barrier.h
@@ -50,6 +50,11 @@
   int relu; float eps, decay; double inv_count;
 };
 
+struct FusedInput {
+  FusedApply f;
+  const float* stats; int rows;
+};
+
 struct FusedBwd {
   unsigned* bar;
   unsigned spin_limit; int fault;
diff --git a/multibox_amd/engine.py b/multibox_amd/engine.py
--- a/multibox_amd/engine.py
+++ b/multibox_amd/engine.py
@@ -155,9 +155,37 @@
         eligible -= drop
 
 
+def fwd_probe(X):
+    d = ops.ConvDesc()
+    d.R, d.S, d.stride, d.epilogue, d.C_in, d.C_out = X.R, X.S, X.stride, ops.EPI_STORE, X.Cin, X.K
+    d.N, d.H_in, d.W_in, d.H_out, d.W_out = X.x.N, X.x.H, X.x.W, X.out.H, X.out.W
+    return d
+
+
+def plan_input_bn(convs, fwd, consumer_ok):
+    is_conv = set(id(c) for c in convs)
+    plan = []
+    for op in convs:
+        u = getattr(op, "unit", None)
+        if op.kind != "bn" or not op.trainable or u is None or len(u.members) != 1 or op.fused_pool is not None:
+            continue
+        buf, lo, hi = op.out.buf, op.out.ch_off, op.out.ch_off + op.K
+        rd = [o for o in fwd if o.x.buf is buf and o.x.ch_off < hi and o.x.ch_off + o.x.C > lo]
+        rd += [o for o in fwd if id(o) in is_conv and o.skip is not None and o.skip.buf is buf and
+               o.skip.ch_off < hi and o.skip.ch_off + o.skip.C > lo]
+        if len(rd) != 1 or id(rd[0]) not in is_conv:
+            continue
+        X = rd[0]
+        if X.kind != "bn" or not X.trainable or len(X.unit.members) != 1 or X.x.buf is not buf or X.x.ch_off != lo or X.x.C != op.K:
+            continue
+        if consumer_ok(X):
+            plan.append((u, X))
+    return plan
+
+
 class Net:
     def __init__(self, batch, input_size=299, k=5, mode="train", fine_tune=False, device="cuda", seed=2,
-                 bn_decay=0.9997, repeats=(10, 20, 9), bn_max_workgroups=0, wgrad_overlap_cus=None):
+                 bn_decay=0.9997, repeats=(10, 20, 9), bn_max_workgroups=0, wgrad_overlap_cus=None, input_bn=None):
         assert mode in ("train", "infer")
         self.repeats = tuple(repeats)
         self.B, self.S, self.k, self.mode, self.fine_tune, self.dev = batch, input_size, k, mode, fine_tune, device
@@ -169,6 +197,9 @@
         self.bw_stats = self.atomic_stats and os.environ.get("MBX_BW_STATS", "0") == "1"
         self.fuse_apply = self.atomic_stats and os.environ.get("MBX_FUSE_APPLY", "0") == "1"
         self.fused_apply_launches = 0
+        self.input_bn = (self.atomic_stats and not self.fuse_apply and torch.device(device).type == "cuda"
+                         and (os.environ["MBX_INPUT_BN"] != "0" if os.environ.get("MBX_INPUT_BN") else input_bn is None or bool(input_bn)))
+        self.input_bn_launches = 0
         self.fuse_bwd = (mode == "train" and not self.deterministic and not self.bw_stats and torch.device(device).type == "cuda"
                          and os.environ.get("MBX_FUSE_BWD", "0") == "1")
         self.fused_bwd_launches = self.fused_bwd_layers = 0
@@ -728,6 +759,13 @@
         L = []
         l = _lib.lib()
         st = lambda: torch.cuda.current_stream().cuda_stream
+        for op in self.convs:
+            op.ibn_from = None
+            if getattr(op, "unit", None) is not None:
+                op.unit.applied_by = None
+        if self.input_bn:
+            for u, X in plan_input_bn(self.convs, self.fwd, lambda X: ops.input_bn_applies(fwd_probe(X))):
+                X.ibn_from = u.lead
         for op in self.fwd:
             if isinstance(op, PoolOp):
                 if not op.fused_fwd:
@@ -777,6 +815,23 @@
         rows = u.rows[i] = ops.conv_stats_rows(d)
         assert use16 or i + 1 == n or rows * op.K * 2 <= u.stats_off[i + 1] - u.stats_off[i]
         u.fwd_desc[i] = d
+        di = bi = prod = None
+        if op.ibn_from is not None and single and use16 and not S_ and cuda and d.tile_config == ops.RESIDENT_TILE_CONFIG:
+            prod, pu = op.ibn_from, op.ibn_from.unit
+            bi = ops.BnInputDesc()
+            bi.stats, bi.rows = self.stats16[pu.stats16_base:].data_ptr(), STATS_ROWS
+            bi.a, bi.ld_a, bi.relu, bi.eps = prod.out.ptr, prod.out.ld, int(prod.relu), BN_EPS
+            bi.beta, bi.mean, bi.rstd, bi.relu_thr = (self._sl(t, prod.beta_off, pu.K).data_ptr() for t in
+                                                      (self.Bt, self.bn_mean, self.bn_rstd, self.bn_thr))
+            di = ops.ConvDesc.from_buffer_copy(d)
+            di.x, di.x_img_stride, di.ldx = prod.y_view.ptr, prod.y_view.img_stride, prod.y_view.ld
+            di.bn_input = C.addressof(bi)
+            if l.mbx_conv_supported(C.byref(di)) == 0:
+                pu.applied_by = op
+                self.input_bn_launches += 1
+                self._keep.append(bi)
+            else:
+                di = bi = prod = None
         if i + 1 < n:
             return lambda: None if u.pair_fwd else _lib.check(l.mbx_conv(C.byref(d), st()), op.name)
         if n == 2 and cuda and os.environ.get("MBX_CONV_PAIR", "1") != "0":
@@ -808,6 +863,9 @@
             else:
                 fd = ba = None
 
+        skip_apply = bool(os.environ.get("MBX_PROBE_SKIP_APPLY")) and single and \
+            re.search(os.environ["MBX_PROBE_SKIP_APPLY"], op.name) is not None
+
         def run():
             s = st()
             mm_, mv_, decay = (None, var, -1.0) if self.defer_moving else (mm, mv, self.bn_decay)
@@ -818,10 +876,17 @@
                 return
             if u.pair_fwd:
                 _lib.check(l.mbx_conv_pair(C.byref(u.fwd_desc[0]), C.byref(d), s), "pair " + op.name)
+            elif di is not None:
+                pmm, pmv, pvar = (self._sl(t, prod.beta_off, prod.unit.K) for t in (self.MM, self.MV, self.bn_var))
+                bi.moving_mean, bi.moving_var, bi.decay = (None, pvar.data_ptr(), -1.0) if self.defer_moving else \
+                    (pmm.data_ptr(), pmv.data_ptr(), self.bn_decay)
+                _lib.check(l.mbx_conv(C.byref(di), s), op.name + " + input bn")
             else:
                 _lib.check(l.mbx_conv(C.byref(d), s), op.name)
             totals = (mean.data_ptr(), rstd.data_ptr(), ops._p(mm_), ops._p(mv_))
-            if use16:
+            if use16 and (skip_apply or u.applied_by is not None):
+                pass
+            elif use16:
                 _lib.check(l.mbx_bn_apply_fused_mapped(s16.data_ptr(), STATS_ROWS, M, BN_EPS, decay, u.y.data_ptr(), M, K,
                                                        beta.data_ptr(), int(op.relu), a_ptr, a_ld, amap, *totals,
                                                        thr.data_ptr(), s), "bn_apply_fused_mapped")
diff --git a/multibox_amd/ops.py b/multibox_amd/ops.py
--- a/multibox_amd/ops.py
+++ b/multibox_amd/ops.py
@@ -32,7 +32,14 @@
         ("relu_bits", C.c_void_p), ("ld_bits", C.c_int32),
         ("bn_apply", C.c_void_p),
         ("bn_bwd", C.c_void_p),
+        ("bn_input", C.c_void_p),
     ]
+
+
+class BnInputDesc(C.Structure):
+    _fields_ = [("stats", C.c_void_p), ("rows", C.c_int32), ("a", C.c_void_p), ("ld_a", C.c_int32), ("beta", C.c_void_p),
+                ("mean", C.c_void_p), ("rstd", C.c_void_p), ("moving_mean", C.c_void_p), ("moving_var", C.c_void_p),
+                ("relu_thr", C.c_void_p), ("relu", C.c_int32), ("eps", C.c_float), ("decay", C.c_float)]
 
 
 class BnApplyDesc(C.Structure):
@@ -246,6 +253,13 @@
     ok = _lib.lib().mbx_conv_supported(C.byref(desc)) == 0
     desc.tile_config = keep
     return ok
+
+
+def input_bn_applies(desc: ConvDesc, min_images=32):
+    taps = desc.R * desc.S
+    if (taps, desc.C_in, desc.C_out) not in ((7, 160, 192), (3, 224, 256)):
+        return False
+    return resident_applies(desc, min_images)
 
 
 PWRES_DEFAULT = "2"
```

After: 4372 images/sec. No clear change (-0.0%).
